# arbobendik/web-ray-tracer

Measured on AMD Instinct MI355X. Metric: Mray/s at 1080p (spp x bounces x pixels / s), higher is better.
Workload: dtype f32

## Files before the change

web-ray-tracer_amd/csrc/flx_api.hip:

```cpp
#include <hip/hip_runtime.h>

#include <chrono>
#include <sched.h>
#include <cstdio>
#include <cstdlib>
#include <algorithm>
#include <cmath>
#include <cstring>
#include <string>
#include <vector>

#include "flx_context.h"

using namespace flx;

#ifndef FLX_FRONT_FUSED_MAX_ITEMS
#define FLX_FRONT_FUSED_MAX_ITEMS (128u << 20)
#endif
#ifndef FLX_FRONT_MIN_TILES_PER_CU
#define FLX_FRONT_MIN_TILES_PER_CU 24
#endif
#ifndef FLX_ADAPTIVE_FRONT_MAX_TILES_PER_CU
#define FLX_ADAPTIVE_FRONT_MAX_TILES_PER_CU 48
#endif
// ... 196 lines not shown
  for (flx_context *c : { ctx, ctx->twin })
    if (c && c->d_frame_rings) (void)hipMemsetAsync(c->d_frame_rings, 0xff, (size_t)c->frame_rings_chains * c->prop.multiProcessorCount * WF_FRAME_RINGS * WF_FRAME_RING * sizeof(uint32_t), c->stream);
  char msg[360];
  snprintf(msg, sizeof msg, "device error in a frame kernel (bits 0x%x:%s%s%s%s%s%s%s): the frame is incomplete", bits, (bits & WF_ERR_SHADE_WATCHDOG) ? " shade-wave watchdog" : "",
           (bits & WF_ERR_WALK_WATCHDOG) ? " walk-wave watchdog" : "", (bits & WF_ERR_LIST) ? " resume list overflow" : "", (bits & WF_ERR_LEFTOVER) ? " paths left behind" : "",
           (bits & WF_ERR_RING_SLOT) ? " ring slot never filled" : "", (bits & WF_ERR_SERVER_IDLE) ? " frame server: nothing to do for seconds" : "",
           (bits & WF_ERR_SERVER_TIMEOUT) ? " frame server: no answer within 5 s" : "");
  std::string full = msg;
  if (ctx->h_sv_mail && (bits & (WF_ERR_SERVER_IDLE | WF_ERR_SERVER_TIMEOUT))) {
    char more[240];
    unsigned long long st[SV_STAT_WORDS] = {};
    if (ctx->d_sv_stats) (void)hipMemcpy(st, ctx->d_sv_stats, sizeof st, hipMemcpyDeviceToHost);
    snprintf(more, sizeof more, " [frame server: posted %u %u %u, done %u %u %u, stop after %u, next %u; launch completed %llu frames, %llu rotations, %llu tiles]", ctx->h_sv_mail->posted[0],
             ctx->h_sv_mail->posted[1], ctx->h_sv_mail->posted[2], ctx->h_sv_mail->done[0], ctx->h_sv_mail->done[1], ctx->h_sv_mail->done[2], ctx->h_sv_mail->stopAfter, ctx->sv_next_seq,
             st[SVS_FRAMES], st[SVS_ROTATIONS], st[SVS_TILES]);
    full += more;
  }
  return flx_fail(ctx, FLX_ERR_DEVICE, full.c_str());
}

static flx_status ensure_workspace(flx_context *ctx, const DeviceFrame &fr, int pipeline, bool counted, int &wf_chains) {
  const size_t P = (size_t)fr.rows * fr.width;
  const uint32_t cus = (uint32_t)ctx->prop.multiProcessorCount;
  wf_chains = 1;
  if (pipeline != 1) {
    flx_status s;
    if (path_item_count64(fr) + 1000000ull >= 4294967296ull) return fail(ctx, FLX_ERR_INVALID, "frame (or batch of frames) too large: more than 2^32 path items");
    {
      const size_t items = (size_t)path_item_count64(fr);
      struct { size_t need, have; } w[] = {
        { P, ctx->d_hits.capacity() }, { P, ctx->d_last.capacity() }, { P * (size_t)fr.samples, ctx->d_samples.capacity() },
        { pipeline == 3 ? items * 8 : 0, ctx->d_rec.capacity() }, { pipeline == 3 ? items * 3 : 0, ctx->d_rec0.capacity() },
        { pipeline == 3 ? items / (size_t)fr.samples * 3 : 0, ctx->d_pix0.capacity() } };
      size_t grow = 0, freed = 0;
      for (auto &b : w) if (b.need > b.have) { grow += b.need * sizeof(float4); freed += b.have * sizeof(float4); }
      if (pipeline == 3) {
        const size_t live = wavefront_live_capacity(fr, cus) * (size_t)(ctx->wf_groups < 1 ? 1 : (ctx->wf_groups > WF_MAX_GROUPS ? WF_MAX_GROUPS : ctx->wf_groups));
        for (auto &list : ctx->d_live) if (!list.fits(live)) { grow += live * sizeof(uint32_t); freed += list.capacity() * sizeof(uint32_t); }
      }
      size_t memFree = 0, memTotal = 0;
      if (grow && hipMemGetInfo(&memFree, &memTotal) == hipSuccess && grow > memFree + freed) {
        char msg[256];
        snprintf(msg, sizeof msg, "the path records of this frame / batch need %.1f GB of device memory, %.1f GB are free (of %.1f GB): render fewer frames per batch or a smaller frame",
                 grow / 1e9, (memFree + freed) / 1e9, memTotal / 1e9);
        return fail(ctx, FLX_ERR_DEVICE, msg);
      }
    }
    if ((s = ctx->d_hits.ensure(ctx, P))) return s;
    if ((s = ctx->d_last.ensure(ctx, P))) return s;
    if ((s = ctx->d_samples.ensure(ctx, P * (size_t)fr.samples))) return s;
  }
  if (pipeline == 3) {
    flx_status s;
    if ((s = ctx->d_rec.ensure(ctx, (size_t)path_item_count(fr) * 8))) return s;
    if ((s = ctx->d_rec0.ensure(ctx, (size_t)path_item_count(fr) * 3))) return s;
    if ((s = ctx->d_pix0.ensure(ctx, (size_t)path_item_count(fr) / (size_t)fr.samples * 3))) return s;
    wf_chains = ctx->wf_groups < 1 ? 1 : (ctx->wf_groups > WF_MAX_GROUPS ? WF_MAX_GROUPS : ctx->wf_groups);
    {
      const uint32_t tiles = path_item_count(fr) / ((uint32_t)fr.samples * 64u);
      if ((uint32_t)wf_chains > tiles || counted) wf_chains = 1;
    }
    const size_t need = wavefront_live_capacity(fr, cus) * (size_t)wf_chains;
    for (auto &list : ctx->d_live) if ((s = list.ensure(ctx, need))) return s;
  }
  return FLX_OK;
}

static flx_status angle_table(flx_context *ctx, DeviceScene &scT) {
  scT.angle_tan = nullptr;
  if (ctx->angle_table && ctx->n_entries != 0u) {
    const uint64_t key = ((uint64_t)ctx->geometry_version << 32) | ctx->transforms_version;
    if (key != ctx->angle_key || !ctx->d_angle_tan) {
      flx_status es = ctx->d_angle_tan.ensure(ctx, ctx->n_entries);
      if (es) return es;
      launch_angle_tan(scT, ctx->d_angle_tan, ctx->stream);
      FLX_HIP(ctx, hipGetLastError());
      ctx->angle_key = key;
    }
    scT.angle_tan = ctx->d_angle_tan;
  }
  return FLX_OK;
}
flx_status flx_angle_table(flx_context *ctx, DeviceScene &sc) { return angle_table(ctx, sc); }

flx_status flx_run_frame(flx_context *ctx, const DeviceScene &sc, const DeviceFrame &fr, float4 *d_out, const GBufferPtrs &gb) {
  { flx_status ss = flx_server_stop(ctx); if (ss) return ss; }
  unsigned long long *cnt = ctx->counters_enabled ? ctx->d_counters : nullptr;
  int pipeline = ctx->pipeline;
  if (pipeline == 0) {
    if (fr.use_filter || fr.is_temporal) pipeline = 1;
    else if (ctx->walk_entries <= 128u) {
      const uint64_t work = (uint64_t)fr.samples * (uint64_t)(fr.max_reflections > 0 ? fr.max_reflections : 1);
      const bool persistent = path_item_count64(fr) >= (1u << 20) && (work >= 32u || (ctx->n_lights >= 4u && work >= 4u));
      pipeline = persistent ? 2 : 1;
    } else pipeline = 3;
  }
  if (pipeline == 3 && fr.max_reflections > WF_MAX_BOUNCES) pipeline = 2;
  ctx->last_pipeline = pipeline;
  ctx->last_organisation = 0;
  ctx->last_trace = TraceKernel{ -1, -1, -1 };
  if (pipeline != 1 && (fr.use_filter || fr.is_temporal)) return fail(ctx, FLX_ERR_INVALID, "pipelines 2 and 3 do not produce the G-buffers of filter / temporal frames");
  const uint32_t cus = (uint32_t)ctx->prop.multiProcessorCount;
  int wf_chains = 1;
  { flx_status s = ensure_workspace(ctx, fr, pipeline, cnt != nullptr, wf_chains); if (s) return s; }
  FLX_HIP(ctx, hipEventRecord(ctx->ev_frame0, ctx->stream));
  if (cnt) FLX_HIP(ctx, hipMemsetAsync(cnt, 0, FLX_COUNTER_SLOTS * sizeof(unsigned long long), ctx->stream));
  if (pipeline == 1) {
    DeviceScene scT = sc;
    { flx_status es = angle_table(ctx, scT); if (es) return es; }
    FLX_HIP(ctx, hipEventRecord(ctx->ev_k0, ctx->stream));
    ctx->last_trace = launch_trace_pixels(scT, fr, d_out, gb, cnt, ctx->stream, ctx->sample_parallel);
    FLX_HIP(ctx, hipGetLastError());
    FLX_HIP(ctx, hipEventRecord(ctx->ev_k1, ctx->stream));
  } else if (pipeline == 2) {
    FLX_HIP(ctx, hipMemsetAsync(ctx->d_queue, 0, sizeof(uint32_t), ctx->stream));
    launch_primary(sc, fr, ctx->d_hits, cnt, ctx->stream);
    FLX_HIP(ctx, hipGetLastError());
    FLX_HIP(ctx, hipEventRecord(ctx->ev_k0, ctx->stream));
    DeviceScene scPaths = sc;
    if (FLX_PATHS_ANGLE_TABLE) { flx_status es = angle_table(ctx, scPaths); if (es) return es; }
    if (ctx->lock_boxes < (uint32_t)FLX_PATHS_LOCK_MIN_BOXES) scPaths.lock_entries = 0u;
    launch_paths(scPaths, fr, ctx->d_hits, ctx->d_samples, ctx->d_last, ctx->d_queue, cus * 8u, cnt, ctx->stream);
    FLX_HIP(ctx, hipGetLastError());
    FLX_HIP(ctx, hipEventRecord(ctx->ev_k1, ctx->stream));
    launch_resolve(fr, ctx->d_hits, ctx->d_samples, ctx->d_last, d_out, ctx->stream);
    FLX_HIP(ctx, hipGetLastError());
  } else {
    FLX_HIP(ctx, hipMemsetAsync(ctx->d_wfcounts, 0, WF_MAX_GROUPS * 2 * (WF_MAX_BOUNCES + 2) * sizeof(uint32_t), ctx->stream));
    { flx_status s = ctx->d_tail_pool.ensure(ctx, (size_t)WF_MAX_GROUPS * cus * 8u * WF_TAIL_POOL_F4); if (s) return s; }
    if (ctx->frame_rings_chains < wf_chains) {
      if (ctx->d_frame_rings) FLX_HIP(ctx, hipStreamSynchronize(ctx->stream));
      ctx->frame_rings_chains = 0;
      const size_t words = (size_t)wf_chains * cus * WF_FRAME_RINGS * WF_FRAME_RING;
      { flx_status s = ctx->d_frame_rings.ensure(ctx, words); if (s) return s; }
      FLX_HIP(ctx, hipMemsetAsync(ctx->d_frame_rings, 0xff, words * sizeof(uint32_t), ctx->stream));
      ctx->frame_rings_chains = wf_chains;
    }
    const int organisationNow = FLX_WF_ORGANISATION_DEFAULT ? FLX_WF_ORGANISATION_DEFAULT : ctx->wf_organisation;
    const uint32_t frameTiles = path_item_count(fr) / ((uint32_t)fr.samples * 64u);
    const int frontMode = wf_chains == 1 ? ctx->frame_front : 0;
    const bool front = (frontMode == 1 || frontMode == 2) && ctx->d_rec0 != nullptr &&
                       (frontMode == 2 || frameTiles >= (uint32_t)FLX_FRONT_MIN_TILES_PER_CU * cus) &&
                       wavefront_front_in_kernel(sc, fr, path_item_count(fr), organisationNow);
    const bool fusedFront = !front && (frontMode == 2 || frontMode == 3 || (frontMode == 1 && path_item_count(fr) <= (uint32_t)FLX_FRONT_FUSED_MAX_ITEMS));
    if (!front && !fusedFront) launch_primary(sc, fr, ctx->d_hits, cnt, ctx->stream);
    FLX_HIP(ctx, hipGetLastError());
    const uint32_t total = path_item_count(fr);
    const uint32_t perTile = (uint32_t)fr.samples * 64u;
    const uint32_t tiles = total / perTile;
    const int groups = wf_chains;
    const bool adaptive = ctx->adaptive_order && (!front || tiles < (uint32_t)FLX_ADAPTIVE_FRONT_MAX_TILES_PER_CU * cus) && groups == 1 && fr.frames <= 1u && !ctx->d_tile_order && cnt == nullptr;
    const int orderMode = 1;
    if (adaptive && !(ctx->d_tile_time.fits(tiles) && ctx->d_auto_order.fits(tiles))) {
      FLX_HIP(ctx, hipStreamSynchronize(ctx->stream));
      ctx->auto_order_tiles = 0;
      flx_status s;
      if ((s = ctx->d_tile_time.ensure(ctx, tiles)) || (s = ctx->d_auto_order.ensure(ctx, tiles))) return s;
    }
    if (adaptive && !(ctx->auto_order_tiles == tiles && ctx->auto_order_width == fr.width && ctx->auto_order_rows == fr.rows && ctx->auto_order_mode == orderMode)) {
      ctx->auto_order_tiles = 0;
      FLX_HIP(ctx, hipMemsetAsync(ctx->d_tile_time, 0, (size_t)tiles * sizeof(float), ctx->stream));
    }
    const size_t listSlice = std::min(ctx->d_live[0].capacity(), ctx->d_live[1].capacity()) / (size_t)groups;
    if (groups > 1) {
      FLX_HIP(ctx, hipEventRecord(ctx->ev_fork, ctx->stream));
      for (int g = 1; g < groups; g++) FLX_HIP(ctx, hipStreamWaitEvent(ctx->aux_stream[g - 1], ctx->ev_fork, 0));
    }
    for (int g = 0; g < groups; g++) {
      const uint32_t t0 = (uint32_t)((uint64_t)tiles * g / groups), t1 = (uint32_t)((uint64_t)tiles * (g + 1) / groups);
      WavefrontBuffers wb;
      wb.rec = ctx->d_rec; wb.rec0 = ctx->d_rec0; wb.pix0 = ctx->d_pix0;
      wb.tailPool = ctx->d_tail_pool + (size_t)g * cus * 8u * WF_TAIL_POOL_F4;
      wb.frameRings = ctx->d_frame_rings + (size_t)g * cus * WF_FRAME_RINGS * WF_FRAME_RING;
      wb.front = front ? 1u : (fusedFront ? 2u : 0u);
      wb.error = ctx->d_dev_error; wb.watchdog = ctx->inject_watchdog; wb.inject = ctx->inject_flags; wb.stampCosts = (adaptive && front) ? 1u : 0u;
      wb.tileOrder = (groups == 1 && ctx->d_tile_order && ctx->tile_order_n == tiles) ? ctx->d_tile_order : nullptr;
      if (!wb.tileOrder && adaptive && ctx->auto_order_tiles == tiles && ctx->auto_order_width == fr.width && ctx->auto_order_rows == fr.rows && ctx->auto_order_mode == orderMode)
        wb.tileOrder = ctx->d_auto_order;
      wb.tileCost = (cnt && ctx->d_tile_cost && ctx->d_tile_cost.capacity() >= tiles) ? ctx->d_tile_cost : nullptr;
      wb.tileCostPrimary = (wb.tileCost && ctx->d_tile_cost.capacity() >= 2u * tiles) ? 1u : 0u;
      wb.live[0] = ctx->d_live[0] + listSlice * g; wb.live[1] = ctx->d_live[1] + listSlice * g;
      wb.counts = ctx->d_wfcounts + (size_t)g * 2 * (WF_MAX_BOUNCES + 2); wb.walkQueue = wb.counts + (WF_MAX_BOUNCES + 2);
      wb.item_base = t0 * perTile; wb.item_count = (t1 - t0) * perTile;
      wb.hits = ctx->d_hits; wb.sampleRadiance = ctx->d_samples; wb.lastOriginal = ctx->d_last; wb.counters = cnt;
      hipStream_t st = g == 0 ? ctx->stream : ctx->aux_stream[g - 1];
      const uint32_t cusWalk = (ctx->comm && (ctx->twin || ctx->is_twin) && cus > 4u * FLX_COMM_RESERVED_CUS) ? cus - FLX_COMM_RESERVED_CUS : cus;
      WalkLdsLaunch lds;
      const int ran = launch_wavefront(sc, fr, wb, cusWalk, cnt != nullptr, organisationNow, g == 0 ? ctx->ev_k0 : nullptr, g == 0 ? ctx->ev_k1 : nullptr, st, &lds);
      FLX_HIP(ctx, hipGetLastError());
      if (ran == -2) return fail(ctx, FLX_ERR_DEVICE, "the walk kernels need 156 KB of dynamic LDS and hipFuncSetAttribute refused it on this device");
      if (ran < 0) return fail(ctx, FLX_ERR_DEVICE, "internal: the frame kernel was to trace the primary rays but does not take this frame");
      ctx->last_organisation = ran;
      ctx->last_walk_lds = lds;
      if (g > 0) {
        FLX_HIP(ctx, hipEventRecord(ctx->ev_join[g - 1], st));
        FLX_HIP(ctx, hipStreamWaitEvent(ctx->stream, ctx->ev_join[g - 1], 0));
      }
    }
    const bool measured = adaptive && ctx->last_organisation >= 2;
    launch_resolve(fr, ctx->d_hits, ctx->d_samples, ctx->d_last, d_out, ctx->stream, 0, measured ? ctx->d_tile_time : nullptr);
    FLX_HIP(ctx, hipGetLastError());
    if (measured) {
      launch_tile_order(ctx->d_tile_time, ctx->d_auto_order, tiles, orderMode, ctx->stream);
      FLX_HIP(ctx, hipGetLastError());
      ctx->auto_order_tiles = tiles; ctx->auto_order_width = fr.width; ctx->auto_order_rows = fr.rows; ctx->auto_order_mode = orderMode;
    } else if (adaptive) ctx->auto_order_tiles = 0;
  }
  FLX_HIP(ctx, hipEventRecord(ctx->ev_frame1, ctx->stream));
  ctx->timed = true;
  return FLX_OK;
}

static flx_status ensure_post_buffers(flx_context *ctx, size_t pixels, bool gbuffers, bool planes);

static flx_status run_post_frame(flx_context *ctx, const DeviceScene &sc, const DeviceFrame &fr, const flx_frame_params *p, float4 *d_out, uint32_t *planes_out = nullptr) {
  const bool temporal = fr.is_temporal == 1, filter = fr.use_filter == 1;
  if (fr.rows != fr.height && (!temporal || (filter && !planes_out)))
    return fail(ctx, FLX_ERR_INVALID, "filter frames cannot be tiled: the denoise chain reads neighbouring pixels (render the whole frame on one context)");
  const size_t pixels = (size_t)fr.rows * fr.width;
  flx_status s;
  if ((s = ensure_post_buffers(ctx, pixels, true, filter && !planes_out))) return s;
  FilterPlanes pl = {};
  if (planes_out) {
    pl.R[0] = planes_out; pl.Ip[0] = planes_out + pixels; pl.O[0] = planes_out + 2 * pixels; pl.Id[0] = planes_out + 3 * pixels; pl.OId = planes_out + 4 * pixels;
  } else if (filter) {
    for (int i = 0; i < 4; i++) { pl.R[i] = ctx->d_planes[i]; pl.Ip[i] = ctx->d_planes[4 + i]; }
    pl.O[0] = ctx->d_planes[8]; pl.O[1] = ctx->d_planes[9]; pl.Id[0] = ctx->d_planes[10]; pl.Id[1] = ctx->d_planes[11]; pl.OId = ctx->d_planes[12];
  }
  int N = 1;
  if (temporal) {
    N = p->temporal_samples <= 0 ? 4 : (p->temporal_samples > 16 ? 16 : p->temporal_samples);
    if (ctx->ring_n != N || ctx->ring_w != fr.width || ctx->ring_h != fr.height ||
        ctx->ring_tile_rows != fr.tile_rows || ctx->ring_tile_index != fr.tile_index || ctx->ring_tile_count != fr.tile_count) {
      ctx->ring_n = 0;
      for (auto &ring : ctx->d_ring) for (auto &plane : ring) if ((s = plane.release(ctx))) return s;
      for (int r = 0; r < 4; r++) for (int i = 0; i < N; i++) {
        if ((s = ctx->d_ring[r][i].ensure(ctx, pixels))) return s;
        FLX_HIP(ctx, hipMemsetAsync(ctx->d_ring[r][i], 0, pixels * sizeof(uint32_t), ctx->stream));
      }
      ctx->ring_n = N; ctx->ring_head = 0; ctx->ring_w = fr.width; ctx->ring_h = fr.height;
      ctx->ring_tile_rows = fr.tile_rows; ctx->ring_tile_index = fr.tile_index; ctx->ring_tile_count = fr.tile_count;
    }
  }
  GBufferPtrs gb = { ctx->d_gb[0], ctx->d_gb[1], ctx->d_gb[2], ctx->d_gb[3], ctx->d_gb[4], ctx->d_gb[5] };
  if (filter && !temporal && !ctx->gb_float_wanted) {
    GBufferPtrs q = { nullptr, nullptr, nullptr, nullptr, nullptr, nullptr };
    q.q_color = pl.R[0]; q.q_color_ip = pl.Ip[0]; q.q_original_color = pl.O[0]; q.q_id = pl.Id[0]; q.q_original_id = pl.OId;
    if ((s = flx_run_frame(ctx, sc, fr, nullptr, q))) return s;
    launch_filter_chain(pl, d_out, (int)fr.width, (int)fr.height, p->hdr, ctx->stream);
    FLX_HIP(ctx, hipGetLastError());
    FLX_HIP(ctx, hipEventRecord(ctx->ev_frame1, ctx->stream));
    return FLX_OK;
  }
  if ((s = flx_run_frame(ctx, sc, fr, nullptr, gb))) return s;
  if (temporal) {
    ctx->ring_head = (ctx->ring_head + N - 1) % N;
    TemporalPass t = {};
    t.color = gb.color; t.color_ip = gb.color_ip; t.location_id = gb.location_id; t.original_id = gb.original_id; t.original_color = gb.original_color; t.id = gb.id;
    for (int k = 0; k < 16; k++) {
      const int slot = (ctx->ring_head + k) % N;
      t.ring_c[k] = k < N ? ctx->d_ring[0][slot] : nullptr; t.ring_ip[k] = k < N ? ctx->d_ring[1][slot] : nullptr;
      t.ring_id[k] = k < N ? ctx->d_ring[2][slot] : nullptr; t.ring_oid[k] = k < N ? ctx->d_ring[3][slot] : nullptr;
    }
    t.n = N; t.hdr = p->hdr; t.pixels = pixels;
    if (filter) { t.dColor = pl.R[0]; t.dIp = pl.Ip[0]; t.dOColor = pl.O[0]; t.dId = pl.Id[0]; t.dOId = pl.OId; }
    else t.out = d_out;
    launch_temporal(t, ctx->stream);
  } else {
    launch_quantize(gb.color, pl.R[0], pixels, ctx->stream);
    launch_quantize(gb.color_ip, pl.Ip[0], pixels, ctx->stream);
    launch_quantize(gb.original_color, pl.O[0], pixels, ctx->stream);
// ... 524 lines not shown
    if ((s = ctx->d_sv_rings.ensure(ctx, ringWords))) return s;
    FLX_HIP(ctx, hipMemsetAsync(ctx->d_sv_rings, 0xff, ringWords * sizeof(uint32_t), ctx->stream));
    if ((s = ctx->d_sv_stats.ensure(ctx, SV_STAT_TOTAL))) return s;
    if ((s = ctx->d_sv_versions.ensure(ctx, (size_t)cus * SV_MAX_DEPTH * SV_BLOB_WORDS))) return s;
    if ((s = ctx->d_sv_slots.ensure(ctx, SV_MAX_DEPTH))) return s;
  }
  int chains = 1;
  if ((s = ensure_workspace(ctx, fr, 3, false, chains))) return s;
  const size_t P1 = (size_t)frOne.rows * frOne.width;
  if (!ctx->sv_target_slots && ctx->d_sv_out.capacity() < SV_MAX_DEPTH * P1) {
    FLX_HIP(ctx, hipStreamSynchronize(ctx->stream));
    if ((s = ctx->d_sv_out.ensure(ctx, SV_MAX_DEPTH * P1))) return s;
  }
  const size_t tilesPerSlot0 = itemsPerSlot / ((size_t)fr.samples * 64u);
  const size_t groupsMin = ctx->sv_groups && ctx->sv_groups < cus ? ctx->sv_groups : (cus > 16 ? cus - 8 : cus);
  size_t tcap = FLX_SERVER_TILE_LIST_FACTOR * (tilesPerSlot0 / groupsMin + 1);
  if (tcap < FLX_SERVER_TILE_LIST_MIN) tcap = FLX_SERVER_TILE_LIST_MIN;
  if (ctx->sv_tile_cap < tcap) {
    ctx->sv_tile_cap = 0;
    if ((s = ctx->d_sv_tiles.ensure(ctx, (size_t)cus * SV_MAX_DEPTH * tcap))) return s;
    ctx->sv_tile_cap = tcap;
  }
  if (!ctx->copy_stream) {
    FLX_HIP(ctx, hipStreamCreateWithFlags(&ctx->copy_stream, hipStreamNonBlocking));
    for (int i = 0; i < 3; i++) {
      FLX_HIP(ctx, hipEventCreate(&ctx->ev_slot_start[i]));
      FLX_HIP(ctx, hipEventCreate(&ctx->ev_slot_traced[i]));
      FLX_HIP(ctx, hipEventCreateWithFlags(&ctx->ev_slot_done[i], hipEventDisableTiming));
    }
  }
  return FLX_OK;
}

static bool server_versions_fit(const flx_context *ctx) {
  return ctx->sv_moving && ctx->have_transforms && ctx->n_transforms != 0 && server_blob_words(ctx->n_transforms, ctx->n_lights) <= SV_BLOB_WORDS &&
         ctx->h_rotation.size() == (size_t)ctx->n_transforms * 24 && ctx->h_shift.size() == (size_t)ctx->n_transforms * 8 && ctx->h_lights.size() == (size_t)ctx->n_lights * 6;
}
static bool server_continues(flx_context *ctx, const flx_frame_params *params, bool out8) {
  const uint32_t depth = ctx->frame_lanes == 3 ? 3u : 2u;
  const bool same_scene = ctx->sv_ver ? ctx->sv_structure_version == ctx->structure_version : ctx->sv_scene_version == ctx->scene_version;
  return ctx->sv_running && ctx->sv_depth == depth && chain_same_shape(ctx->sv_params, *params) && same_scene && ctx->sv_out8 == out8;
}
int flx_server_takes_moving_scene(const flx_context *ctx) { return ctx->sv_want_ver && server_versions_fit(ctx) ? 1 : 0; }
int flx_server_continues(flx_context *ctx, const flx_frame_params *params) { return server_continues(ctx, params, ctx->sv_target_slots != 0u && ctx->sv_target8) ? 1 : 0; }
flx_status flx_server_prepare(flx_context *ctx, const flx_frame_params *params) {
  FLX_HIP(ctx, hipSetDevice(ctx->device));
  DeviceScene sc; DeviceFrame fr;
  flx_status s = flx_make_frame(ctx, params, sc, fr);
  if (s) return s;
  if ((s = flx_server_stop(ctx))) return s;
  if (ctx->sv_stream) FLX_HIP(ctx, hipStreamSynchronize(ctx->sv_stream));
  if ((s = server_allocate(ctx, fr, ctx->frame_lanes == 3 ? 3u : 2u))) return s;
  FLX_HIP(ctx, hipStreamSynchronize(ctx->stream));
  return FLX_OK;
}

static flx_status server_post(flx_context *ctx, const flx_frame_params *params, const DeviceScene &sc, const DeviceFrame &frOne, uint32_t *seqOut, uint32_t *slotOut, bool out8) {
  const uint32_t cus = (uint32_t)ctx->prop.multiProcessorCount;
  const uint32_t depth = ctx->frame_lanes == 3 ? 3u : 2u;
  flx_status s;
  if (ctx->sv_running && !server_continues(ctx, params, out8))
    if ((s = server_stop(ctx))) return s;
  if (ctx->sv_running && server_idled_with_nothing_owed(ctx)) {
    ctx->sv_running = false;
    FLX_HIP(ctx, hipStreamSynchronize(ctx->sv_stream));
    __atomic_store_n(&ctx->h_dev_error[0], 0u, __ATOMIC_RELEASE);
  }
  if (!ctx->sv_running) {
    if ((s = flx_dyn_flush(ctx))) return s;
    if (ctx->sv_stream) FLX_HIP(ctx, hipStreamSynchronize(ctx->sv_stream));
    if (server_idled_with_nothing_owed(ctx)) __atomic_store_n(&ctx->h_dev_error[0], 0u, __ATOMIC_RELEASE);
    for (int i = 0; i < ctx->fifo_n; i++) {
      if (ctx->fifo[i].lane != ctx) continue;
      const int kp = ctx->fifo[i].slot;
      if (ctx->sv_pending[kp].valid && (s = server_take(ctx, kp))) return s;
    }
    DeviceFrame fr = frOne;
    fr.frames = depth; fr.rows = depth * frOne.frame_rows;
    for (uint32_t i = 0; i < depth; i++) memset(&fr.view[i], 0, sizeof(FrameView));
    const size_t itemsPerSlot = (size_t)path_item_count64(frOne);
    if ((s = server_allocate(ctx, frOne, depth))) return s;
    const size_t P1 = (size_t)frOne.rows * frOne.width;
    ctx->sv_out_pixels = P1;
    FLX_HIP(ctx, hipStreamSynchronize(ctx->stream));
    ctx->sv_counter += 16u;
    if (ctx->sv_counter < 16u) ctx->sv_counter = 16u;
    const uint32_t seq0 = ctx->sv_counter;
    memset((void *)ctx->h_sv_mail, 0, sizeof(ServerMail));
    FLX_HIP(ctx, hipMemsetAsync(ctx->d_sv_slots, 0, SV_MAX_DEPTH * sizeof(ServerSlot), ctx->sv_stream));
    FLX_HIP(ctx, hipMemsetAsync(ctx->d_sv_relay, 0, sizeof(ServerMail), ctx->sv_stream));
    FLX_HIP(ctx, hipMemsetAsync(ctx->d_sv_stats, 0, SV_STAT_TOTAL * sizeof(unsigned long long), ctx->sv_stream));
    WavefrontBuffers wb = {};
    wb.rec = ctx->d_rec; wb.rec0 = ctx->d_rec0; wb.pix0 = ctx->d_pix0;
    wb.frameRings = ctx->d_sv_rings; wb.front = 1u;
    wb.error = ctx->d_dev_error; wb.watchdog = 0u; wb.inject = 0u;
    wb.item_base = 0u; wb.item_count = (uint32_t)(depth * itemsPerSlot);
    wb.hits = ctx->d_hits; wb.sampleRadiance = ctx->d_samples; wb.lastOriginal = ctx->d_last; wb.counters = nullptr;
    ServerArgs sa = {};
    sa.slots = ctx->d_sv_slots; sa.mail = ctx->d_sv_mail; sa.relay = ctx->d_sv_relay;
    const uint32_t slot0 = ctx->sv_target_slots ? (uint32_t)(ctx->sv_target_posted % depth) : ((ctx->fifo_n && ctx->sv_depth == depth) ? ctx->sv_next_slot % depth : 0u);
    sa.depth = depth; sa.slot0 = slot0; sa.seq0 = seq0;
    sa.tilesPerSlot = (uint32_t)(itemsPerSlot / ((size_t)fr.samples * 64u));
    sa.itemsPerSlot = (uint32_t)itemsPerSlot;
    for (uint32_t i = 0; i < depth; i++) sa.out[i] = ctx->d_sv_out + (size_t)i * P1;
    if (ctx->sv_target_slots) {
      const size_t first = (size_t)params->tile_index * params->tile_rows * params->width;
      for (uint32_t i = 0; i < depth; i++) sa.out[i] = out8 ? (float4 *)((uint32_t *)ctx->sv_target[i] + first) : ctx->sv_target[i] + first;
      sa.outStripRows = params->tile_rows; sa.outStripStep = params->tile_rows * params->tile_count; sa.outSystem = 1u;
    }
    sa.out8 = out8 ? 1u : 0u;
    sa.tileLists = ctx->d_sv_tiles; sa.tileListCap = (uint32_t)ctx->sv_tile_cap;
    sa.idleExit = 200000000u;
    sa.error = ctx->d_dev_error;
    sa.stats = ctx->d_sv_stats;
    uint32_t cusWalk = cus > 4u * FLX_SERVER_RESERVED_CUS ? cus - FLX_SERVER_RESERVED_CUS : cus;
    if (ctx->sv_groups && ctx->sv_groups < cusWalk) cusWalk = ctx->sv_groups;
    const bool ver = ctx->sv_want_ver && server_versions_fit(ctx);
    DeviceScene scL = sc;
    if (ver) {
      const size_t versions = (size_t)cusWalk * depth;
      sa.blobWords = server_blob_words(ctx->n_transforms, ctx->n_lights);
      scL.rotation = (const float4 *)ctx->d_sv_versions.get();
      scL.shift = (const float4 *)(ctx->d_sv_versions + versions * ctx->n_transforms * 24u);
      scL.lights = (const float *)(ctx->d_sv_versions + versions * ctx->n_transforms * 32u);
    }
    if (launch_server(scL, fr, wb, sa, cusWalk, ctx->sv_stream, &ctx->last_walk_lds) != 0) return fail(ctx, FLX_ERR_DEVICE, "internal: the frame server does not take this scene");
    FLX_HIP(ctx, hipGetLastError());
    ctx->sv_running = true; ctx->sv_depth = depth; ctx->sv_next_seq = seq0; ctx->sv_next_slot = slot0;
    ctx->sv_params = *params; ctx->sv_scene_version = ctx->scene_version; ctx->sv_out8 = out8;
    ctx->sv_ver = ver; ctx->sv_structure_version = ctx->structure_version;
  }
  const uint32_t seq = ctx->sv_next_seq++, slot = ctx->sv_next_slot;
  ctx->sv_next_slot = (slot + 1u) % depth;
  if (ctx->sv_target_slots) ctx->sv_target_posted++;
  memcpy((void *)&ctx->h_sv_mail->view[slot], &frOne.view[0], sizeof(FrameView));
  if (ctx->sv_ver) {
    uint32_t *b = (uint32_t *)ctx->h_sv_mail->blob[slot];
    memcpy(b, ctx->h_rotation.data(), (size_t)ctx->n_transforms * 96);
    memcpy(b + (size_t)ctx->n_transforms * 24, ctx->h_shift.data(), (size_t)ctx->n_transforms * 32);
    if (ctx->n_lights) memcpy(b + (size_t)ctx->n_transforms * 32, ctx->h_lights.data(), (size_t)ctx->n_lights * 24);
  }
  __atomic_store_n(&ctx->h_sv_mail->posted[slot], seq, __ATOMIC_RELEASE);
  *seqOut = seq; *slotOut = slot;
  ctx->last_pipeline = 3; ctx->last_organisation = 5; ctx->last_chained = 3; ctx->last_trace = TraceKernel{ -1, -1, -1 };
  return FLX_OK;
}

static flx_status server_take(flx_context *ctx, int k) {
  auto &pf = ctx->sv_pending[k];
  pf.valid = false;
  ctx->slot_latency_ms[k] = -1.f;
  const auto t0 = std::chrono::steady_clock::now();
  uint32_t spins = 0;
  while (__atomic_load_n(&ctx->h_sv_mail->done[pf.slot], __ATOMIC_ACQUIRE) != pf.seq) {
    if (__atomic_load_n(&ctx->h_dev_error[0], __ATOMIC_ACQUIRE) != 0u) break;
    if ((++spins & 1023u) == 0u && std::chrono::steady_clock::now() - t0 > std::chrono::seconds(5)) {
      __atomic_fetch_or(&ctx->h_dev_error[0], WF_ERR_SERVER_TIMEOUT, __ATOMIC_RELEASE);
      break;
    }
    if (spins < 4096u) __builtin_ia32_pause(); else sched_yield();
  }
  if (server_idled_with_nothing_owed(ctx)) {
    ctx->sv_running = false;
    FLX_HIP(ctx, hipStreamSynchronize(ctx->sv_stream));
    __atomic_store_n(&ctx->h_dev_error[0], 0u, __ATOMIC_RELEASE);
  }
  if (__atomic_load_n(&ctx->h_dev_error[0], __ATOMIC_ACQUIRE) != 0u) {
    __atomic_store_n(&ctx->h_sv_mail->stopAfter, 1u, __ATOMIC_RELEASE);
    ctx->sv_running = false;
    return FLX_OK;
  }
  ctx->slot_latency_ms[k] = std::chrono::duration<float, std::milli>(std::chrono::steady_clock::now() - pf.posted).count();
  const float4 *src = ctx->sv_target_slots ? ctx->sv_target[pf.slot] : ctx->d_sv_out + (size_t)pf.slot * ctx->sv_out_pixels;
  ctx->slot_dev_ptr[k] = src;
  FLX_HIP(ctx, hipEventRecord(ctx->ev_slot_start[k], ctx->copy_stream));
  FLX_HIP(ctx, hipEventRecord(ctx->ev_slot_traced[k], ctx->copy_stream));
  if (pf.format != FLX_FRAME_DEVICE) {
    if (ctx->slot_bytes[k]) FLX_HIP(ctx, hipMemcpyAsync(ctx->h_slot[k], src, ctx->slot_bytes[k], hipMemcpyDeviceToHost, ctx->copy_stream));
    FLX_HIP(ctx, hipEventRecord(ctx->ev_slot_done[k], ctx->copy_stream));
  }
  return FLX_OK;
}

constexpr int NOT_GATHERED = -2;
struct FrameKind { bool raster = false; int aa = 0;  };
static flx_status frame_begin_on(flx_context *ctx, const flx_frame_params *params, int format, int gather, int *slot, int chained = 0 ,
                                 FrameKind kind = FrameKind()) {
  FLX_HIP(ctx, hipSetDevice(ctx->device));
  DeviceScene sc; DeviceFrame fr;
  flx_status s = flx_make_frame(ctx, params, sc, fr);
  if (s) return s;
  if (!chained) ctx->last_chained = 0;
  const bool gathered = gather != NOT_GATHERED;
  const bool receiver = !gathered || gather < 0 || gather == ctx->comm_rank;
  if (gathered) { fr.rows = receiver ? params->height : 0u; }
  const int k = (int)(ctx->frames_begun % (uint64_t)(ctx->frame_lanes == 3 ? 3 : 2));
  if (!ctx->copy_stream) {
    FLX_HIP(ctx, hipStreamCreateWithFlags(&ctx->copy_stream, hipStreamNonBlocking));
    for (int i = 0; i < 3; i++) {
      FLX_HIP(ctx, hipEventCreate(&ctx->ev_slot_start[i]));
      FLX_HIP(ctx, hipEventCreate(&ctx->ev_slot_traced[i]));
// ... 572 lines not shown
```

web-ray-tracer_amd/csrc/flx_context.h:

```cpp
#ifndef FLX_CONTEXT_H
#define FLX_CONTEXT_H

#include <hip/hip_runtime.h>

#include <chrono>
#include <cstdint>
#include <string>
#include <vector>

#include "flexlight_hip.h"
#include "flexlight_hip_debug.h"
#include "flx_kernels.h"
#include "flx_ray_temporal_args.h"
#include "flx_server.h"

struct flx_share;
typedef struct ncclComm *flx_nccl_comm;

#ifndef FLX_WF_GROUPS
#define FLX_WF_GROUPS 1
#endif
constexpr int WF_MAX_GROUPS = 4;
#ifndef FLX_SAMPLE_PARALLEL_DEFAULT
#define FLX_SAMPLE_PARALLEL_DEFAULT 1
// ... 20 lines not shown
  T *operator->() const { return p; }
  size_t capacity() const { return n; }
  bool fits(size_t count) const { return p && n >= count; }
  flx_status ensure(flx_context *ctx, size_t count, unsigned pinned_flags = 0);
  flx_status release(flx_context *ctx);
  void borrow(const Buffer &o) { (void)hip_free(); p = o.p; n = o.n; owned = false; }
 private:
  T *p = nullptr;
  size_t n = 0;
  bool owned = true;
  hipError_t hip_free() {
    T *mine = owned ? p : nullptr;
    p = nullptr; n = 0; owned = true;
    return !mine ? hipSuccess : Pinned ? hipHostFree(mine) : hipFree(mine);
  }
};
template <typename T> using DeviceBuffer = Buffer<T, false>;
template <typename T> using PinnedBuffer = Buffer<T, true>;

struct flx_context {
  int device = 0;
  hipStream_t own_stream = nullptr, stream = nullptr;
  std::string err;
  hipDeviceProp_t prop;
  DeviceBuffer<float4> d_geometry, d_attributes, d_rotation, d_shift;
  DeviceBuffer<float4> d_walk;
  uint32_t walk_entries = 0, walk_hot = 0, walk_root = 0, walk_fast_boxes = 0;
  uint32_t walk_thick_boxes = 0;
  int box_test = -1;
  DeviceBuffer<float4> d_fwd;
  uint32_t fwd_entries = 0, fwd_root = 0, lock_boxes = 0;
  int last_organisation = 0;
  flx::WalkLdsLaunch last_walk_lds;
  int frame_front = 1;
  DeviceBuffer<uint32_t> d_frame_rings;
  int frame_rings_chains = 0;
  int wf_organisation = 0;
  bool lock_ok = false;
  bool lock_use = true;
  bool gb_float_wanted = false;
  int sample_parallel = FLX_SAMPLE_PARALLEL_DEFAULT;
  int adaptive_order = 1;
  DeviceBuffer<float> d_tile_time; DeviceBuffer<uint32_t> d_auto_order;
  uint32_t auto_order_tiles = 0, auto_order_width = 0, auto_order_rows = 0; int auto_order_mode = -1;
  DeviceBuffer<uint32_t> d_tile_order; uint32_t tile_order_n = 0;
  DeviceBuffer<unsigned long long> d_tile_cost;
  DeviceBuffer<int32_t> d_ids;
  DeviceBuffer<float> d_lights;
  DeviceBuffer<uchar4> d_atlas[3];
  uint32_t atlas_w[3] = { 0, 0, 0 }, atlas_h[3] = { 0, 0, 0 };
  struct { uint32_t w = 0, h = 0, n = 0; } atlas_cells[3];
  DeviceBuffer<flx::AtlasSource> d_texture_table;
  DeviceBuffer<uint4> d_texture_src;
  DeviceBuffer<uint32_t> d_texture_cell;
  uint32_t n_entries = 0, n_ids = 0, n_transforms = 0, n_lights = 0;
  uint32_t max_transform = 0;
  bool have_scene = false, have_transforms = false, have_lights = false;
  std::vector<uint32_t> h_entry_meta;
  bool scene_has_nan = false;
  PinnedBuffer<float> h_update;
  hipEvent_t update_done = nullptr;
  bool update_pending = false;
  DeviceBuffer<float4> d_update_rows, d_update_attributes;
  DeviceBuffer<uint32_t> d_update_verdict;
  PinnedBuffer<uint32_t> h_update_verdict;
  hipStream_t update_stream = nullptr;
  hipEvent_t update_checked = nullptr, update_produced = nullptr, geometry_uploaded = nullptr;
  DeviceBuffer<uint32_t> d_refit;
  DeviceBuffer<uint32_t> d_derive;
  PinnedBuffer<uint32_t> h_derive_record;
  bool entry_meta_stale = false;
  struct {
    DeviceBuffer<float2> tbox; DeviceBuffer<uint32_t> perm[2], owner[2], open, bucket, entry, keys, verdict, refit; DeviceBuffer<uint2> x, y, totals;
    DeviceBuffer<uint4> node, cnt; DeviceBuffer<double> centre;
    size_t node_capacity = 0;
    uint32_t n_triangles = 0, n_nodes = 0; int current = 0; float transform = 0.0f; bool valid = false;
  } tree;
  PinnedBuffer<uint32_t> h_tree_record;
  DeviceBuffer<float4> d_angle_tan;
  uint64_t angle_key = ~0ull;
  uint32_t geometry_version = 0;
  uint32_t transforms_version = 0;
  int angle_table = 1;
  DeviceBuffer<float4> d_out;
  DeviceBuffer<float4> d_gb[6];
  DeviceBuffer<uint32_t> d_planes[13];
  DeviceBuffer<uint32_t> d_qbatch;
  DeviceBuffer<uint32_t> d_ring[4][16];
  int ring_n = 0, ring_head = 0;
  uint32_t ring_w = 0, ring_h = 0;
  uint32_t ring_tile_rows = 0, ring_tile_index = 0, ring_tile_count = 0;
  DeviceBuffer<float4> d_hits, d_samples, d_last;
  DeviceBuffer<uint32_t> d_queue;
  DeviceBuffer<float4> d_rec;
  DeviceBuffer<float4> d_tail_pool;
  DeviceBuffer<uint32_t> d_aa[10];
  uint32_t aa_w = 0, aa_h = 0;
  int taa_head = 0, taa_filled = 0;
  DeviceBuffer<float4> d_aa_io[2];
  DeviceBuffer<float4> d_rec0, d_pix0;
  DeviceBuffer<uint32_t> d_live[2];
  DeviceBuffer<uint32_t> d_wfcounts;
  int pipeline = 0;
  int last_pipeline = 0;
  flx::TraceKernel last_trace = { -1, -1, -1 };
  int wf_groups = FLX_WF_GROUPS;
  hipStream_t aux_stream[3] = { nullptr, nullptr, nullptr };
  hipEvent_t ev_fork = nullptr, ev_join[3] = { nullptr, nullptr, nullptr };
  PinnedBuffer<uint32_t> h_dev_error; uint32_t *d_dev_error = nullptr;
  uint32_t inject_watchdog = 0, inject_flags = 0;
  DeviceBuffer<unsigned long long> d_counters;
  bool counters_enabled = false;
  flx_counters last_counters = {};
  hipEvent_t ev_frame0 = nullptr, ev_frame1 = nullptr, ev_k0 = nullptr, ev_k1 = nullptr;
  bool timed = false;
  flx_nccl_comm comm = nullptr;
  flx_nccl_comm comm_twin = nullptr;
  int last_gather_root = -1;
  int comm_rank = 0, comm_size = 1;
  bool comm_owned = false;
  DeviceBuffer<float4> d_send, d_recv;
  DeviceBuffer<float4> d_send8;
  DeviceBuffer<float4> d_frames;
  DeviceBuffer<float4> d_gplanes;
  DeviceBuffer<float4> d_slot[3];
  DeviceBuffer<uint32_t> d_slot8[3];
  PinnedBuffer<uint8_t> h_slot[3];
  size_t slot_bytes[3] = { 0, 0, 0 };
  hipStream_t copy_stream = nullptr;
  hipEvent_t ev_slot_start[3] = {}, ev_slot_traced[3] = {}, ev_slot_done[3] = {};
  uint64_t frames_begun = 0, frames_ended = 0;
  bool slot_host[3] = { true, true, true };
  flx_context *twin = nullptr;
  bool is_twin = false;
  int frame_lanes = 2;
  uint64_t lane_next = 0;
  struct { flx_context *lane; int slot; } fifo[3] = {};
  int fifo_n = 0;
  std::vector<float> h_lights, h_rotation, h_shift;
  uint64_t dyn_version = 0, twin_dyn_version = 0;
  int frame_chain = FLX_FRAME_CHAIN_DEFAULT;
  uint64_t scene_version = 0;
  uint64_t begin_scene_version = 0;
  int last_chained = 0;
  DeviceBuffer<flx::ServerSlot> d_sv_slots;
  PinnedBuffer<flx::ServerMail> h_sv_mail; flx::ServerMail *d_sv_mail = nullptr;
  DeviceBuffer<flx::ServerMail> d_sv_relay;
  DeviceBuffer<uint32_t> d_sv_rings;
  DeviceBuffer<float4> d_sv_out;
  size_t sv_out_pixels = 0;
  DeviceBuffer<uint32_t> d_sv_tiles;
  size_t sv_tile_cap = 0;
  float slot_latency_ms[3] = { -1.f, -1.f, -1.f };
  const void *slot_dev_ptr[3] = { nullptr, nullptr, nullptr };
  DeviceBuffer<unsigned long long> d_sv_stats;
  hipStream_t sv_stream = nullptr;
  bool sv_running = false;
  uint32_t sv_depth = 0, sv_next_seq = 0, sv_next_slot = 0, sv_counter = 0;
  flx_frame_params sv_params = {};
  uint64_t sv_scene_version = 0;
  uint64_t structure_version = 0;
  uint64_t sv_structure_version = 0;
  bool sv_ver = false;
  uint32_t dyn_device_stale = 0;
  bool sv_want_ver = false;
  int sv_moving = 1;
// ... 105 lines not shown
```

web-ray-tracer_amd/csrc/flx_device.h:

```cpp
#ifndef FLX_DEVICE_H
#define FLX_DEVICE_H

#include <hip/hip_runtime.h>
#include <stdint.h>

#include "flx_math.h"

#define FLX_DEV __device__ __forceinline__

namespace flx {

constexpr float PHI = 1.61803398874989484820459f;
constexpr float SQRT3 = 1.7320508075688772f;
constexpr float INV_PI = 0.3183098861837907f;
constexpr float INV_256 = 0.00390625f;
constexpr float INV_255 = 0.00392156862745098f;
constexpr float PI_F = 3.141592653589793f;
constexpr float BIAS = FLX_BIAS;
constexpr float POW32 = FLX_POW32;
constexpr float NEAR_VIEW_DEPTH = 0.5f;

struct f3 { float x, y, z; };
struct f4 { float x, y, z, w; };
struct M3 { f3 c0, c1, c2; };

FLX_DEV f3 F3(float x, float y, float z) { f3 r; r.x = x; r.y = y; r.z = z; return r; }
FLX_DEV f3 operator+(f3 a, f3 b) { return F3(a.x + b.x, a.y + b.y, a.z + b.z); }
FLX_DEV f3 operator-(f3 a, f3 b) { return F3(a.x - b.x, a.y - b.y, a.z - b.z); }
FLX_DEV f3 operator*(f3 a, f3 b) { return F3(a.x * b.x, a.y * b.y, a.z * b.z); }
FLX_DEV f3 operator/(f3 a, f3 b) { return F3(a.x / b.x, a.y / b.y, a.z / b.z); }
FLX_DEV f3 operator*(f3 a, float s) { return F3(a.x * s, a.y * s, a.z * s); }
FLX_DEV f3 operator/(f3 a, float s) { return F3(a.x / s, a.y / s, a.z / s); }
FLX_DEV f3 operator-(f3 a) { return F3(-a.x, -a.y, -a.z); }
FLX_DEV float dot(f3 a, f3 b) { return (a.x * b.x + a.y * b.y) + a.z * b.z; }
FLX_DEV f3 cross(f3 a, f3 b) { return F3(a.y * b.z - b.y * a.z, a.z * b.x - b.z * a.x, a.x * b.y - b.x * a.y); }
FLX_DEV float length(f3 a) { return flx_sqrt(dot(a, a)); }
FLX_DEV f3 normalize(f3 a) { return a / length(a); }
FLX_DEV float distance(f3 a, f3 b) { return length(a - b); }
FLX_DEV f3 mix(f3 a, f3 b, float t) { return F3(flx_mix(a.x, b.x, t), flx_mix(a.y, b.y, t), flx_mix(a.z, b.z, t)); }
FLX_DEV f3 mul(const M3 &m, f3 v) {
  return F3((m.c0.x * v.x + m.c1.x * v.y) + m.c2.x * v.z,
            (m.c0.y * v.x + m.c1.y * v.y) + m.c2.y * v.z,
            (m.c0.z * v.x + m.c1.z * v.y) + m.c2.z * v.z);
}
FLX_DEV f3 reflect(f3 I, f3 N) { return I - N * (2.0f * dot(N, I)); }
FLX_DEV f3 refract(f3 I, f3 N, float eta) {
  float d = dot(N, I);
  float k = 1.0f - eta * eta * (1.0f - d * d);
  if (k < 0.0f) return F3(0.0f, 0.0f, 0.0f);
  return I * eta - N * (eta * d + flx_sqrt(k));
}

struct Ray { f3 origin, dir; };
struct Material { f3 albedo, rme, tpo; };
struct Hit { f3 suv; int transformId; int triangleId; };

struct DeviceScene {
  const float4 *geometry;
  const float4 *attributes;
  const float4 *rotation;
  const float4 *shift;
  const float *lights;
  const uchar4 *atlas[3];
  uint32_t atlas_w[3], atlas_h[3];
  uint32_t n_entries;
  uint32_t n_lights;
  uint32_t n_transforms;
  uint32_t walk_thick_boxes;
  const float4 *walk;
  uint32_t walk_entries;
  uint32_t walk_hot;
  uint32_t walk_root;
  uint32_t walk_fast_boxes;
  const float4 *lock;
  uint32_t lock_entries;
  uint32_t lock_root;
  const float4 *fwd;
  uint32_t fwd_entries, fwd_root;
  const float4 *angle_tan;
};
#ifndef FLX_LOCKSTEP
#define FLX_LOCKSTEP 1
#endif
#define FLX_LOCK_MAX 128u
constexpr uint32_t WALK_END = 0x30000000u;
constexpr uint32_t LINK_INDEX = 0x0fffffffu, LINK_XFORM = 0x40000000u;
constexpr int LINK_KIND_SHIFT = 28;
FLX_DEV uint32_t linkIndex(uint32_t link) { return link & LINK_INDEX; }
FLX_DEV uint32_t linkKind(uint32_t link) { return (link >> LINK_KIND_SHIFT) & 3u; }
// ... 172 lines not shown
  if (!(s < l) || !(s * viewDepthPerS >= NEAR_VIEW_DEPTH)) return false;
  suv = F3(s, u, v);
  return s != 0.0f;
}

FLX_DEV bool rayCuboid(float l, const Ray &ray, f3 minCorner, f3 maxCorner) {
  f3 v0 = (minCorner - ray.origin) / ray.dir;
  f3 v1 = (maxCorner - ray.origin) / ray.dir;
  float tmin = flx_max(flx_max(flx_min(v0.x, v1.x), flx_min(v0.y, v1.y)), flx_min(v0.z, v1.z));
  float tmax = flx_min(flx_min(flx_max(v0.x, v1.x), flx_max(v0.y, v1.y)), flx_max(v0.z, v1.z));
  return tmax >= flx_max(tmin, BIAS) && tmin < l;
}

FLX_DEV float trowbridgeReitz(float alpha, float NdotH) {
  float numerator = alpha * alpha;
  float denom = NdotH * NdotH * (numerator - 1.0f) + 1.0f;
  return numerator / flx_max(PI_F * denom * denom, BIAS);
}
FLX_DEV float schlickBeckmann(float alpha, float NdotX) {
  float k = alpha * 0.5f;
  float denominator = NdotX * (1.0f - k) + k;
  denominator = flx_max(denominator, BIAS);
  return NdotX / denominator;
}
FLX_DEV float smith(float alpha, float NdotV, float NdotL) { return schlickBeckmann(alpha, NdotV) * schlickBeckmann(alpha, NdotL); }
FLX_DEV f3 fresnel(f3 F0, float theta) {
  float p = flx_pow5(1.0f - theta);
  return F3(F0.x + (1.0f - F0.x) * p, F0.y + (1.0f - F0.y) * p, F0.z + (1.0f - F0.z) * p);
}

FLX_DEV f3 forwardTrace(const Material &material, f3 lightDir, float strength, f3 N, f3 V) {
  float lenP1 = 1.0f + length(lightDir);
  float brightness = strength / (lenP1 * lenP1);
  f3 L = normalize(lightDir);
  f3 H = normalize(V + L);
  float VdotH = flx_max(dot(V, H), 0.0f);
  float NdotL = flx_max(dot(N, L), 0.0f);
  float NdotH = flx_max(dot(N, H), 0.0f);
  float NdotV = flx_max(dot(N, V), 0.0f);
  float alpha = material.rme.x * material.rme.x;
  float BRDF = flx_mix(1.0f, NdotV, material.rme.y);
  f3 F0 = material.albedo * BRDF;
  f3 Ks = fresnel(F0, VdotH);
  float oneMinusMetal = 1.0f - material.rme.y;
  f3 Kd = F3((1.0f - Ks.x) * oneMinusMetal, (1.0f - Ks.y) * oneMinusMetal, (1.0f - Ks.z) * oneMinusMetal);
  f3 lambert = material.albedo * INV_PI;
  float tr = trowbridgeReitz(alpha, NdotH);
  float sm = smith(alpha, NdotV, NdotL);
  f3 cookTorranceNumerator = (Ks * tr) * sm;
  float cookTorranceDenominator = 4.0f * NdotV * NdotL;
  cookTorranceDenominator = flx_max(cookTorranceDenominator, BIAS);
  f3 cookTorrance = cookTorranceNumerator / cookTorranceDenominator;
  f3 radiance = Kd * lambert + cookTorrance;
  return (radiance * NdotL) * brightness;
}

struct PixelState {
  float firstRayLength, glassFilter, originalRMEx, originalTPOx;
  f3 originalColor;
  f4 renderId, renderOriginalId;
  float ndc_x, ndc_y;
  float seed;
  uint32_t lightBase = 0;
};

struct PathState {
  Ray ray;
  f3 lastHitPoint;
  f3 finalColor, importancyFactor;
  Hit hit;
  bool dontFilter;
};

struct ShadeOut {
  f3 litColor;
  f3 baseLuminance;
  Ray shadowRay;
  float shadowLen;
  bool needShadow;
  bool shadowedNoWalk;
  bool markId;
};

FLX_DEV void reservoirPick(const DeviceScene &sc, const DeviceFrame &fr, PixelState &ps, const Material &material, const Ray &ray,
                           f4 randomVec, f3 N, f3 smoothNormal, float geometryOffset, bool dontFilter, int i, ShadeOut &so) {
  f3 localColor = F3(0.0f, 0.0f, 0.0f);
  float reservoirLength = 0.0f;
  float totalWeight = 0.0f;
  int reservoirNum = 0;
  float reservoirWeight = 0.0f;
  f3 reservoirLightDir = F3(0.0f, 0.0f, 0.0f);
  f4 n0 = noise(ps.seed, randomVec.z, randomVec.w, BIAS);
  float lastRandomX = n0.x, lastRandomY = n0.y;
  const int size = (int)sc.n_lights;
  for (int j = 0; j < size; j++) {
    const float *lt = sc.lights + 6 * j + ps.lightBase;
    float strength = lt[3], variation = lt[4];
    if (strength <= 0.0f) continue;
    reservoirLength += 1.0f;
    f3 light = F3(lt[0], lt[1], lt[2]) + F3(randomVec.x, randomVec.y, randomVec.z) * variation;
    f3 dir = light - ray.origin;
    f3 colorForLight = forwardTrace(material, dir, strength, N, -ray.dir);
    localColor = localColor + colorForLight;
    float weight = length(colorForLight);
    totalWeight += weight;
    if (flx_abs(lastRandomY) * totalWeight <= weight) {
      reservoirNum = j;
      reservoirWeight = weight;
      reservoirLightDir = dir;
    }
    if (j + 1 < size) {
      f4 n1 = noise(ps.seed, lastRandomX, lastRandomY, BIAS);
      lastRandomX = n1.z; lastRandomY = n1.w;
    }
  }
  f3 unitLightDir = normalize(reservoirLightDir);
  bool showColor = reservoirLength == 0.0f || reservoirWeight == 0.0f;
  bool showShadow = dot(smoothNormal, unitLightDir) <= BIAS;
  so.baseLuminance = F3(material.rme.z, material.rme.z, material.rme.z);
  so.litColor = localColor + so.baseLuminance;
  so.markId = dontFilter || i == 0;
  if (so.markId) ps.renderId.w = (float)((reservoirNum % 128) << 1) * INV_255;
  so.needShadow = !showColor && !showShadow;
  so.shadowedNoWalk = !showColor && showShadow;
  so.shadowRay.origin = ray.origin + smoothNormal * geometryOffset;
  so.shadowRay.dir = unitLightDir;
  so.shadowLen = length(reservoirLightDir);
}

struct SurfaceCtx {
  f3 origin;
  f3 dir;
  f3 smoothNormal;
  float signDir, geometryOffset, BRDF, roughnessBRDF;
  f3 F0;
  Material material;
};

#ifndef FLX_ANGLE_TABLE
#define FLX_ANGLE_TABLE 0
#endif
FLX_DEV f3 triangleAngleTan(f3 t0v, f3 t1v, f3 t2v, f3 n0, f3 n1, f3 n2) {
  f3 geometryNormal = normalize(cross(t0v - t1v, t0v - t2v));
  f3 angles = F3(flx_acos(flx_abs(dot(geometryNormal, n0))), flx_acos(flx_abs(dot(geometryNormal, n1))),
                 flx_acos(flx_abs(dot(geometryNormal, n2))));
  return F3(flx_clamp(flx_tan(angles.x), 0.0f, 1.0f), flx_clamp(flx_tan(angles.y), 0.0f, 1.0f),
            flx_clamp(flx_tan(angles.z), 0.0f, 1.0f));
}
FLX_DEV f3 triangleAngleTanOf(const DeviceScene &sc, int tri) {
  const float4 g0 = sc.geometry[3 * tri], g1 = sc.geometry[3 * tri + 1], g2 = sc.geometry[3 * tri + 2];
  const M3 rTI = rotation_at(sc, (int)g2.y << 1);
  const float4 *at = sc.attributes + 7 * (size_t)tri;
  const float4 a0 = at[0], a1 = at[1], a2 = at[2];
  return triangleAngleTan(mul(rTI, F3(g0.x, g0.y, g0.z)), mul(rTI, F3(g0.w, g1.x, g1.y)), mul(rTI, F3(g1.z, g1.w, g2.x)),
                          mul(rTI, F3(a0.x, a0.y, a0.z)), mul(rTI, F3(a0.w, a1.x, a1.y)), mul(rTI, F3(a1.z, a1.w, a2.x)));
}

template <bool COUNT>
FLX_DEV void shadeSurface(const DeviceScene &sc, const DeviceFrame &fr, const Hit &hit, const Ray &ray, f3 lastHitPoint, SurfaceCtx &sf,
                          WorkCounters &cnt) {
  if (COUNT) cnt.shades++;
  M3 rTI = rotation_at(sc, hit.transformId);
  f3 sTI = shift_at(sc, hit.transformId);
  sf.origin = ray.dir * hit.suv.x + ray.origin;
  f3 uvw = F3(1.0f - hit.suv.y - hit.suv.z, hit.suv.y, hit.suv.z);
  float4 g0 = sc.geometry[3 * hit.triangleId], g1 = sc.geometry[3 * hit.triangleId + 1], g2 = sc.geometry[3 * hit.triangleId + 2];
  f3 t0v = mul(rTI, F3(g0.x, g0.y, g0.z));
  f3 t1v = mul(rTI, F3(g0.w, g1.x, g1.y));
  f3 t2v = mul(rTI, F3(g1.z, g1.w, g2.x));
  f3 offsetRayTarget = sf.origin - sTI;
  f3 diffs = F3(distance(offsetRayTarget, t0v), distance(offsetRayTarget, t1v), distance(offsetRayTarget, t2v));
  const float4 *at = sc.attributes + 7 * (size_t)hit.triangleId;
  float4 a0 = at[0], a1 = at[1], a2 = at[2], a3 = at[3], a4 = at[4], a5 = at[5], a6 = at[6];
  f3 n0 = mul(rTI, F3(a0.x, a0.y, a0.z));
  f3 n1 = mul(rTI, F3(a0.w, a1.x, a1.y));
  f3 n2 = mul(rTI, F3(a1.z, a1.w, a2.x));
  f3 smoothNormal = normalize(F3((n0.x * uvw.x + n1.x * uvw.y) + n2.x * uvw.z,
                                 (n0.y * uvw.x + n1.y * uvw.y) + n2.y * uvw.z,
                                 (n0.z * uvw.x + n1.z * uvw.y) + n2.z * uvw.z));
  f3 angleTan;
  if (FLX_ANGLE_TABLE && sc.angle_tan) { const float4 t = sc.angle_tan[hit.triangleId]; angleTan = F3(t.x, t.y, t.z); }
  else angleTan = triangleAngleTan(t0v, t1v, t2v, n0, n1, n2);
  sf.geometryOffset = dot(diffs * angleTan, uvw);
  float bu = (a2.y * uvw.x + a2.w * uvw.y) + a3.y * uvw.z;
  float bv = (a2.z * uvw.x + a3.x * uvw.y) + a3.z * uvw.z;
  sf.material.albedo = fetchTexVal<COUNT>(sc, fr, 0, bu, bv, a3.w, F3(a4.z, a4.w, a5.x), cnt);
  sf.material.rme = fetchTexVal<COUNT>(sc, fr, 1, bu, bv, a4.x, F3(a5.y, a5.z, a5.w), cnt);
  sf.material.tpo = fetchTexVal<COUNT>(sc, fr, 2, bu, bv, a4.y, F3(a6.x, a6.y, a6.z), cnt);

  sf.dir = normalize(sf.origin - lastHitPoint);
  sf.signDir = flx_sign(dot(sf.dir, smoothNormal));
  sf.smoothNormal = smoothNormal * (-sf.signDir);
  sf.BRDF = flx_mix(1.0f, flx_abs(dot(sf.smoothNormal, sf.dir)), sf.material.rme.y);
  sf.roughnessBRDF = sf.material.rme.x * sf.BRDF;
  sf.F0 = sf.material.albedo * sf.BRDF;
}

FLX_DEV void shadeSample(const DeviceScene &sc, const DeviceFrame &fr, const SurfaceCtx &sf, PixelState &ps, PathState &p, f3 camera, float cosSampleN,
                         int i, ShadeOut &so) {
  const float fi = (float)i;
  const Material &material = sf.material;
  const f3 smoothNormal = sf.smoothNormal;
  p.ray.origin = sf.origin;
  p.ray.dir = sf.dir;
  f4 randomVec = noise(ps.seed, ps.ndc_x, ps.ndc_y, fi + cosSampleN);
  f3 randomSpheareVec = normalize(smoothNormal + normalize(F3(randomVec.x, randomVec.y, randomVec.z)));
  f3 roughNormal = normalize(mix(smoothNormal, randomSpheareVec, sf.roughnessBRDF));
  f3 H = normalize(roughNormal - p.ray.dir);
  float VdotH = flx_max(dot(-p.ray.dir, H), 0.0f);
  f3 f = fresnel(sf.F0, VdotH);
  float fresnelReflect = flx_max(f.x, flx_max(f.y, f.z));
  bool isSolid = material.tpo.x * fresnelReflect <= flx_abs(randomVec.w);

  if (p.dontFilter) {
    ps.originalTPOx = material.tpo.x;
    ps.originalColor = ps.originalColor * material.albedo;
    ps.originalRMEx += material.rme.x;
    if (fr.use_filter) {
      float scale = flx_exp2_neg_int(i);
      f3 cn = combineNormalRME(smoothNormal, material.rme);
      f4 upd; upd.x = scale * cn.x; upd.y = scale * cn.y; upd.z = scale * cn.z; upd.w = scale * 0.0f;
      ps.renderId.x += upd.x; ps.renderId.y += upd.y; ps.renderId.z += upd.z; ps.renderId.w += upd.w;
      if (i == 0) {
        ps.renderOriginalId.x += upd.x; ps.renderOriginalId.y += upd.y; ps.renderOriginalId.z += upd.z; ps.renderOriginalId.w += upd.w;
      }
    }
    p.dontFilter = (material.rme.x < 0.01f && isSolid) || !isSolid;
    if (isSolid && material.tpo.x > 0.01f) {
      ps.glassFilter += 1.0f;
      p.dontFilter = false;
    }
  } else {
    p.importancyFactor = p.importancyFactor * material.albedo;
  }

  if (i == 1) ps.firstRayLength = flx_min(length(p.ray.origin - p.lastHitPoint) / length(p.lastHitPoint - camera), ps.firstRayLength);
  reservoirPick(sc, fr, ps, material, p.ray, randomVec, roughNormal * (-sf.signDir), smoothNormal * (-sf.signDir), sf.geometryOffset, p.dontFilter, i, so);
  if (isSolid) {
    p.ray.dir = normalize(mix(reflect(p.ray.dir, smoothNormal), randomSpheareVec, sf.roughnessBRDF));
  } else {
    float eta = flx_mix(1.0f / material.tpo.z, material.tpo.z, flx_max(sf.signDir, 0.0f));
    p.ray.dir = normalize(mix(refract(p.ray.dir, smoothNormal, eta), randomSpheareVec, sf.roughnessBRDF));
  }
}

template <bool COUNT>
FLX_DEV void bounceShade(const DeviceScene &sc, const DeviceFrame &fr, PixelState &ps, PathState &p, f3 camera, float cosSampleN, int i,
                         ShadeOut &so, WorkCounters &cnt) {
  SurfaceCtx sf;
  shadeSurface<COUNT>(sc, fr, p.hit, p.ray, p.lastHitPoint, sf, cnt);
  shadeSample(sc, fr, sf, ps, p, camera, cosSampleN, i, so);
}

#ifndef FLX_BOX_FALLBACK_COUNT
#define FLX_BOX_FALLBACK_COUNT 0
#endif
struct WalkState {
  Ray src;
  Ray tR;
  float minLen;
  int i;
  int cachedTI;
  int mode;
  int shadowed;
  f3 suv;
  int tri, hitTI;
  f3 inv;
  bool fastDiv;
#if FLX_BOX_FALLBACK_COUNT
  mutable uint32_t boxTests, boxExact;
#endif
};

FLX_DEV void walkStart(WalkState &w, int mode, const Ray &ray, float len) {
  w.mode = mode; w.src = ray; w.tR = ray; w.cachedTI = 0; w.minLen = len; w.i = 0;
}
FLX_DEV void walkClearResults(WalkState &w) {
  w.inv = F3(0.0f, 0.0f, 0.0f); w.fastDiv = false;
  w.shadowed = false; w.suv = F3(0.0f, 0.0f, 0.0f); w.tri = -1; w.hitTI = 0;
}

template <bool COUNT>
FLX_DEV bool walkStep(const DeviceScene &sc, WalkState &w, WorkCounters &cnt) {
  bool endWalk = false;
  const int i = w.i;
  float4 e0 = sc.geometry[3 * i], e1 = sc.geometry[3 * i + 1], e2 = sc.geometry[3 * i + 2];
  if (COUNT) { if (w.mode == 0) cnt.shadow_visits++; else cnt.closest_visits++; }
  int tI = (int)e2.y << 1;
  if (tI != w.cachedTI) {
    int iI = tI + 1;
    M3 rotationII = rotation_at(sc, iI);
    w.cachedTI = tI;
    w.tR.origin = mul(rotationII, w.src.origin + shift_at(sc, iI));
    f3 d = mul(rotationII, w.src.dir);
    w.tR.dir = (w.mode == 0) ? normalize(d) : d;
  }
  int next = i + 1;
  if (e2.z == 0.0f) {
    endWalk = true;
  } else if (e2.z == 1.0f) {
    if (!rayCuboid(w.minLen, w.tR, F3(e0.x, e0.y, e0.z), F3(e0.w, e1.x, e1.y))) next += (int)e1.z;
  } else {
    f3 a = F3(e0.x, e0.y, e0.z), b = F3(e0.w, e1.x, e1.y), c = F3(e1.z, e1.w, e2.x);
    if (w.mode == 0) {
      if (moellerTrumboreCull(a, b, c, w.tR, w.minLen)) { w.shadowed = true; endWalk = true; }
    } else {
      f3 suv;
      if (moellerTrumbore(a, b, c, w.tR, w.minLen, suv)) {
        w.suv = suv; w.hitTI = tI; w.tri = i;
        w.minLen = suv.x;
      }
    }
  }
  w.i = next;
  return endWalk || next >= (int)sc.n_entries;
}

struct WalkEntry { float4 e0, e1, e2; };


FLX_DEV float divByRecip(float a, float d, float y) {
  float q = a * y;
  float r = __builtin_fmaf(-q, d, a);
  q = __builtin_fmaf(r, y, q);
  r = __builtin_fmaf(-q, d, a);
  return __builtin_fmaf(r, y, q);
}
FLX_DEV void reciprocalOfDir(const DeviceScene &sc, f3 d, f3 o, f3 &inv, bool &fast) {
  inv = F3(recipFast(d.x), recipFast(d.y), recipFast(d.z));
  const float LO = 8.673617379884035e-19f, HI = 1.152921504606847e18f, OHI = 5.764607523034235e17f;
  const float ax = flx_abs(d.x), ay = flx_abs(d.y), az = flx_abs(d.z);
  fast = sc.walk_fast_boxes != 0u && ax >= LO && ax <= HI && ay >= LO && ay <= HI && az >= LO && az <= HI &&
         flx_abs(o.x) <= OHI && flx_abs(o.y) <= OHI && flx_abs(o.z) <= OHI;
}
// ... 584 lines not shown
```

web-ray-tracer_amd/csrc/flx_frame_common.h:

```cpp
#pragma once
#include "flx_kernels.h"
#include "flx_kernel_util.h"
#include "flx_wavefront_common.h"

namespace flx {

#ifndef FLX_WF_WALK_THREADS
#define FLX_WF_WALK_THREADS 1024
#endif
#ifndef FLX_WF_WAVES_PER_EU
#define FLX_WF_WAVES_PER_EU 4
#endif
#ifndef FLX_WF_LDS_TOTAL
#define FLX_WF_LDS_TOTAL (156 * 1024)
#endif
#ifndef FLX_WF_INNER
#define FLX_WF_INNER 8
#endif
#ifndef FLX_WF_UNROLL
#define FLX_WF_UNROLL 8
#endif
#ifndef FLX_WF_BATCH
#define FLX_WF_BATCH 24
#endif
#ifndef FLX_WF_DRAWS_PER_WAVE
#define FLX_WF_DRAWS_PER_WAVE 16
#endif
#ifndef FLX_FRAME_SHADERS_FRONT
#define FLX_FRAME_SHADERS_FRONT 4
#endif
#ifndef FLX_WF_MAX_TRANSFORMS
#define FLX_WF_MAX_TRANSFORMS 4
#endif
#ifndef FLX_FRAME_PROLOGUE_WAVES
#define FLX_FRAME_PROLOGUE_WAVES 2
#endif
#ifndef FLX_FRAME_READY_UNITS
#define FLX_FRAME_READY_UNITS 32
#endif

typedef const __attribute__((address_space(4))) FrameArgs *FrameArgsP;
FLX_DEV const FrameArgs &frame_args(FrameArgsP p) { asm volatile("" : "+s"(p)); return *(const FrameArgs *)p; }
FLX_DEV FrameArgsP kernel_frame_args() { return (FrameArgsP)__builtin_amdgcn_kernarg_segment_ptr(); }
#define FLX_ARGS_OF(ab) const FrameArgs &A_ = frame_args(ab); const DeviceScene &sc = A_.sc; const DeviceFrame &fr = A_.fr; const WavefrontBuffers &wb = A_.wb; (void)sc; (void)fr; (void)wb

template <bool VER>
FLX_DEV uint32_t scene_version_of(const DeviceFrame &fr, uint32_t frameIdx) { return VER ? blockIdx.x * fr.frames + frameIdx : 0u; }

template <bool COUNT, bool LV = false, bool VER = false>
FLX_DEV bool shade0_tile(FrameArgsP ab, uint32_t tile, uint32_t lane, float4 h, WorkCounters &cnt, const FrameView *lv = nullptr) {
  uint32_t S, frameIdx, lightBase = 0;
  int tri;
  bool alive, compact;
  f3 camera;
  SurfaceCtx sf;
  float ndcX = 0.0f, ndcY = 0.0f;
  Hit hit;
  {
  FLX_ARGS_OF(ab);
  S = (uint32_t)fr.samples;
  uint32_t px, k;
  tile8_pixel(fr, tile, lane, px, k);
  const bool inFrame = px < fr.width && k < fr.rows;
  frameIdx = inFrame ? frame_index(fr, k) : 0u;
  camera = view_camera(view_at<LV>(fr, lv, frameIdx));
  tri = inFrame ? __float_as_int(h.w) : -1;
  alive = tri != -1 && fr.max_reflections > 0 && length(F3(1.0f, 1.0f, 1.0f) * F3(1.0f, 1.0f, 1.0f)) >= fr.min_importancy * SQRT3;
  hit.suv = F3(h.x, h.y, h.z); hit.triangleId = tri; hit.transformId = 0;
  compact = wb.rec0 != nullptr;
  if (alive) {
    hit.transformId = (int)sc.geometry[3 * tri + 2].y << 1;
    if (VER) { const uint32_t ver = scene_version_of<VER>(fr, frameIdx); hit.transformId += (int)(ver * 2u * sc.n_transforms); lightBase = ver * 6u * sc.n_lights; }
    const uint32_t py_gl = fr.height - 1u - image_row(fr, k);
    float viewDepthPerS;
    Ray pr;
    pr.origin = camera;
    pr.dir = primary_dir_v(fr, view_at<LV>(fr, lv, frameIdx), px, py_gl, ndcX, ndcY, viewDepthPerS);
    const WorkCounters before = cnt;
    shadeSurface<COUNT>(sc, fr, hit, pr, camera, sf, cnt);
    if (COUNT) {
      cnt.shades = before.shades + (cnt.shades - before.shades) * S;
      cnt.atlas_texels = before.atlas_texels + (cnt.atlas_texels - before.atlas_texels) * S;
    }
  }
  }
  for (uint32_t s = 0; s < S; s++) {
    FLX_ARGS_OF(ab);
    const uint32_t pathId = ((tile * S + s) << 6) | lane;
    float4 *rec = wb.rec + (size_t)pathId * 8;
    if (!alive) {
      if (tri != -1) finalize_path<LV>(fr, wb, pathId, F3(0.0f, 0.0f, 0.0f), F3(1.0f, 1.0f, 1.0f), F3(1.0f, 1.0f, 1.0f), lv);
      if (compact) wb.rec0[(size_t)pathId * 3] = make_float4(0.f, 0.f, 0.f, __int_as_float(RF_DEAD));
      else rec[0] = make_float4(0.f, 0.f, 0.f, __int_as_float(RF_DEAD));
      continue;
    }
    PathState p;
    PixelState ps;
    ps.firstRayLength = 1.0f; ps.glassFilter = 0.0f; ps.originalRMEx = 0.0f; ps.originalTPOx = 0.0f;
    ps.renderId.x = ps.renderId.y = ps.renderId.z = ps.renderId.w = 0.0f;
    ps.renderOriginalId = ps.renderId;
    ps.ndc_x = ndcX; ps.ndc_y = ndcY;
    ps.seed = view_at<LV>(fr, lv, frameIdx).random_seed;
    ps.lightBase = lightBase;
    ps.originalColor = F3(1.0f, 1.0f, 1.0f);
    p.hit = hit;
    p.lastHitPoint = camera;
    p.dontFilter = true;
    p.importancyFactor = F3(1.0f, 1.0f, 1.0f);
    const float cosSampleN = flx_cos((float)s);
    ShadeOut so;
    shadeSample(sc, fr, sf, ps, p, camera, cosSampleN, 0, so);
    const int flags = (p.dontFilter ? RF_DONT_FILTER : 0) | (so.needShadow ? RF_NEED_SHADOW : 0) | (so.shadowedNoWalk ? RF_SHADOWED_NO_WALK : 0) |
                      (nextBounceRuns(fr, 0, p.importancyFactor, ps.originalColor) ? 0 : RF_NO_CLOSEST);
    if (compact) {
      if (s == 0u) {
        float4 *pp = wb.pix0 + (((size_t)tile << 6) | lane) * 3;
        pp[0] = make_float4(p.ray.origin.x, p.ray.origin.y, p.ray.origin.z, 0.0f);
        pp[1] = make_float4(so.shadowRay.origin.x, so.shadowRay.origin.y, so.shadowRay.origin.z, 0.0f);
        pp[2] = make_float4(ps.originalColor.x, ps.originalColor.y, ps.originalColor.z, so.baseLuminance.x);
      }
      float4 *r0 = wb.rec0 + (size_t)pathId * 3;
      r0[0] = make_float4(p.ray.dir.x, p.ray.dir.y, p.ray.dir.z, __int_as_float(flags));
      r0[1] = make_float4(so.shadowRay.dir.x, so.shadowRay.dir.y, so.shadowRay.dir.z, so.shadowLen);
      r0[2] = make_float4(so.litColor.x, so.litColor.y, so.litColor.z, 0.0f);
      continue;
    }
    rec[0] = make_float4(p.ray.origin.x, p.ray.origin.y, p.ray.origin.z, __int_as_float(flags));
    rec[1] = make_float4(p.ray.dir.x, p.ray.dir.y, p.ray.dir.z, so.shadowLen);
    rec[2] = make_float4(so.shadowRay.origin.x, so.shadowRay.origin.y, so.shadowRay.origin.z, so.baseLuminance.x);
    rec[3] = make_float4(so.shadowRay.dir.x, so.shadowRay.dir.y, so.shadowRay.dir.z, __int_as_float(0));
    rec[4] = make_float4(so.litColor.x, so.litColor.y, so.litColor.z, 0.0f);
    rec[5] = make_float4(0.0f, 0.0f, 0.0f, 0.0f);
    rec[6] = make_float4(p.importancyFactor.x, p.importancyFactor.y, p.importancyFactor.z, 0.0f);
    rec[7] = make_float4(ps.originalColor.x, ps.originalColor.y, ps.originalColor.z, 0.0f);
  }
  return alive;
}

template <bool COUNT, bool LV = false, bool VER = false>
FLX_DEV float4 primary_tile(FrameArgsP ab, uint32_t tile, uint32_t lane, WorkCounters &cnt, const FrameView *lv = nullptr) {
  FLX_ARGS_OF(ab);
  float4 *__restrict__ hits = const_cast<float4 *>(wb.hits);
  uint32_t px, k;
  tile8_pixel(fr, tile, lane, px, k);
  const bool inImage = px < fr.width && k < fr.rows;
  float nx, ny, viewDepthPerS = 0.0f;
  Ray pr; pr.origin = F3(0.0f, 0.0f, 0.0f); pr.dir = F3(0.0f, 0.0f, 1.0f);
  int xfBase = 0;
  if (inImage) {
    const uint32_t py_gl = fr.height - 1u - image_row(fr, k);
    const uint32_t frameIdx = frame_index(fr, k);
    if (VER) xfBase = (int)(scene_version_of<VER>(fr, frameIdx) * 2u * sc.n_transforms);
    const FrameView &v = view_at<LV>(fr, lv, frameIdx);
    pr.dir = primary_dir_v(fr, v, px, py_gl, nx, ny, viewDepthPerS);
    pr.origin = view_camera(v);
  }
  const uint32_t visitsBefore = cnt.primary_visits;
  const Hit hp = primaryWalkF(sc, inImage, pr, viewDepthPerS, cnt.primary_visits, xfBase);
  if (COUNT && wb.tileCost && wb.tileCostPrimary) {
    const uint32_t nTiles = ((fr.width + 7u) >> 3) * ((fr.rows + 7u) >> 3);
    atomicAdd(wb.tileCost + nTiles + tile, (unsigned long long)(cnt.primary_visits - visitsBefore));
  }
  float4 h = make_float4(hp.suv.x, hp.suv.y, hp.suv.z, __int_as_float(inImage ? hp.triangleId : -1));
  if (inImage) {
    if (COUNT && hp.triangleId != -1) cnt.primary_hits++;
    hits[(size_t)k * fr.width + px] = h;
  }
  return h;
}

template <bool COUNT, bool LV = false, bool VER = false>
FLX_DEV void shade_path(FrameArgsP ab, uint32_t pathId, WorkCounters &cnt, const FrameView *lv = nullptr) {
  FLX_ARGS_OF(ab);
  float4 *rec = wb.rec + (size_t)pathId * 8;
  uint32_t px, k, s;
  item_pixel(fr, pathId, px, k, s);
  const uint32_t frameIdx = frame_index(fr, k);
  const f3 camera = view_camera(view_at<LV>(fr, lv, frameIdx));
  PathState p;
  PixelState ps;
  ps.firstRayLength = 1.0f; ps.glassFilter = 0.0f; ps.originalRMEx = 0.0f; ps.originalTPOx = 0.0f;
  ps.renderId.x = ps.renderId.y = ps.renderId.z = ps.renderId.w = 0.0f;
  ps.renderOriginalId = ps.renderId;
  const float4 q0 = rec[0], q1 = rec[1], q2 = rec[2], q3 = rec[3], q6 = rec[6], q7 = rec[7];
  const int pb = __float_as_int(q3.w) + 1;
  p.ray.origin = F3(q0.x, q0.y, q0.z);
  p.lastHitPoint = p.ray.origin;
  p.ray.dir = F3(q1.x, q1.y, q1.z);
  p.hit.suv = F3(q2.x, q2.y, q2.z);
  p.hit.triangleId = __float_as_int(q2.w);
  p.hit.transformId = (int)sc.geometry[3 * p.hit.triangleId + 2].y << 1;
  if (VER) { const uint32_t ver = scene_version_of<VER>(fr, frameIdx); p.hit.transformId += (int)(ver * 2u * sc.n_transforms); ps.lightBase = ver * 6u * sc.n_lights; }
  p.dontFilter = (__float_as_int(q0.w) & RF_DONT_FILTER) != 0;
  p.importancyFactor = F3(q6.x, q6.y, q6.z);
  ps.originalColor = F3(q7.x, q7.y, q7.z);
  const uint32_t py_gl = fr.height - 1u - image_row(fr, k);
  float viewDepthPerS;
  (void)primary_dir_v(fr, view_at<LV>(fr, lv, frameIdx), px, py_gl, ps.ndc_x, ps.ndc_y, viewDepthPerS);
  ps.seed = view_at<LV>(fr, lv, frameIdx).random_seed;
  const float cosSampleN = flx_cos((float)s);
  ShadeOut so;
  bounceShade<COUNT>(sc, fr, ps, p, camera, cosSampleN, pb, so, cnt);
  const int flags = (p.dontFilter ? RF_DONT_FILTER : 0) | (so.needShadow ? RF_NEED_SHADOW : 0) | (so.shadowedNoWalk ? RF_SHADOWED_NO_WALK : 0) |
                    (nextBounceRuns(fr, pb, p.importancyFactor, ps.originalColor) ? 0 : RF_NO_CLOSEST);
  rec[0] = make_float4(p.ray.origin.x, p.ray.origin.y, p.ray.origin.z, __int_as_float(flags));
  rec[1] = make_float4(p.ray.dir.x, p.ray.dir.y, p.ray.dir.z, so.shadowLen);
  rec[2] = make_float4(so.shadowRay.origin.x, so.shadowRay.origin.y, so.shadowRay.origin.z, so.baseLuminance.x);
  rec[3] = make_float4(so.shadowRay.dir.x, so.shadowRay.dir.y, so.shadowRay.dir.z, __int_as_float(pb));
  rec[4] = make_float4(so.litColor.x, so.litColor.y, so.litColor.z, 0.0f);
  rec[6] = make_float4(p.importancyFactor.x, p.importancyFactor.y, p.importancyFactor.z, 0.0f);
  rec[7] = make_float4(ps.originalColor.x, ps.originalColor.y, ps.originalColor.z, 0.0f);
}

struct WalkLane {
  int st;
  uint32_t pathId; int flags; int pathBounce; float base;
  Ray nextRay, shadowRay; float shadowLen;
  WalkState w; WalkEntry cur;
  uint32_t v0;
};
FLX_DEV void walkLaneInit(WalkLane &L) {
  L.v0 = 0u;
  L.st = P_EMPTY; L.pathId = 0; L.flags = 0; L.pathBounce = 0; L.base = 0.0f;
  L.nextRay.origin = F3(0.f, 0.f, 0.f); L.nextRay.dir = L.nextRay.origin;
  L.shadowRay = L.nextRay; L.shadowLen = 0.0f;
  walkClearResults(L.w);
  L.w.src = L.nextRay; L.w.tR = L.nextRay; L.w.minLen = 0.0f; L.w.i = 0; L.w.cachedTI = 0;
  L.w.mode = 2;
  L.cur.e0 = L.cur.e1 = L.cur.e2 = make_float4(0.f, 0.f, 0.f, 0.f);
}
FLX_DEV const float4 *pix_part(const DeviceFrame &fr, const WavefrontBuffers &wb, uint32_t id) {
  uint32_t tile0, s0;
  item_tile(fr, id, tile0, s0);
  return wb.pix0 + (((size_t)tile0 << 6) | (id & 63u)) * 3;
}
#ifndef FLX_WF_FOLD_EARLY
#define FLX_WF_FOLD_EARLY 1
#endif
#if FLX_WF_FOLD_EARLY
struct WalkFold { float4 q4, q5, q6, q7; bool compact; };
#define FLX_WALK_LANE_FOLD_FETCH(fr_, wb_, compactRecs_, L_, F_)                                                                 \
  do {                                                                                                                           \
    const float4 *a4_ = (wb_).rec + (size_t)(L_).pathId * 8 + 4, *a7_ = a4_ + 3;                                                 \
    (F_).compact = (compactRecs_) && (L_).pathBounce == 0;                                                                       \
    if ((F_).compact) { a4_ = (wb_).rec0 + (size_t)(L_).pathId * 3 + 2; a7_ = pix_part(fr_, wb_, (L_).pathId) + 2; }             \
     \
    (F_).q4 = *a4_; (F_).q7 = *a7_;                                                                                              \
    if (!(F_).compact) { (F_).q5 = a4_[1]; (F_).q6 = a4_[2]; }       \
  } while (0)
#define FLX_WALK_LANE_FOLD_WITH(LV_, fr_, wb_, compactRecs_, L_, F_, lv_, toShade_, ended_, costed_, stamp_)                     \
  do {                                                                                                                           \
    float4 *rec_ = (wb_).rec + (size_t)(L_).pathId * 8;                                                                          \
    const bool compact_ = (F_).compact;                                                                                          \
    const float4 q4_ = (F_).q4, q7_ = (F_).q7;                                                                                   \
    float4 q5_ = make_float4(0.0f, 0.0f, 0.0f, 0.0f), q6_ = make_float4(1.0f, 1.0f, 1.0f, 0.0f);                                 \
    if (!compact_) { q5_ = (F_).q5; q6_ = (F_).q6; }                                                                             \
    const bool shadowed_ = ((L_).flags & RF_SHADOWED_NO_WALK) || (((L_).flags & RF_NEED_SHADOW) && (L_).w.shadowed);            \
    const f3 localColor_ = shadowed_ ? F3((L_).base, (L_).base, (L_).base) : F3(q4_.x, q4_.y, q4_.z);                            \
    const f3 importancy_ = F3(q6_.x, q6_.y, q6_.z), originalColor_ = F3(q7_.x, q7_.y, q7_.z);                                    \
    const f3 finalColor_ = F3(q5_.x, q5_.y, q5_.z) + localColor_ * importancy_;                                                  \
     \
    const float cost_ = (costed_) ? q5_.w + (float)(((stamp_) - ((uint32_t)(L_).flags >> 8)) & 0xffffffu) : 1.0f;      \
    bool cont_ = (L_).w.tri != -1;                                                                                               \
    if (cont_) cont_ = ((L_).pathBounce + 1) < (fr_).max_reflections && length(importancy_ * originalColor_) >= (fr_).min_importancy * SQRT3;      \
    if (cont_) {                                                                                                                 \
      if (compact_) {                                         \
                                                                            \
        rec_[0] = make_float4((L_).nextRay.origin.x, (L_).nextRay.origin.y, (L_).nextRay.origin.z, __int_as_float((L_).flags & 0xff));             \
        rec_[1] = make_float4((L_).nextRay.dir.x, (L_).nextRay.dir.y, (L_).nextRay.dir.z, (L_).shadowLen);                                         \
        rec_[3] = make_float4((L_).shadowRay.dir.x, (L_).shadowRay.dir.y, (L_).shadowRay.dir.z, __int_as_float(0));                                \
        rec_[6] = make_float4(1.0f, 1.0f, 1.0f, 0.0f);                                                                           \
        rec_[7] = make_float4(q7_.x, q7_.y, q7_.z, 0.0f);                                                                        \
      }                                                                                                                          \
      rec_[5] = make_float4(finalColor_.x, finalColor_.y, finalColor_.z, (costed_) ? cost_ : 0.0f);                                                 \
      rec_[2] = make_float4((L_).w.suv.x, (L_).w.suv.y, (L_).w.suv.z, __int_as_float((L_).w.tri));                               \
      toShade_ = true;                                                                                                           \
    } else {                                                                                                                     \
      finalize_path<LV_>(fr_, wb_, (L_).pathId, finalColor_, importancy_, originalColor_, lv_, cost_);                           \
      ended_ = true;                                                                                                             \
    }                                                                                                                            \
    (L_).st = P_EMPTY;                                                                                                           \
  } while (0)
#define FLX_WALK_LANE_FOLD(LV_, fr_, wb_, compactRecs_, L_, lv_, toShade_, ended_, costed_, stamp_)                              \
  do {                                                                                                                           \
    WalkFold fold_;                                                                                                              \
// ... 194 lines not shown
```

web-ray-tracer_amd/csrc/flx_kernels.h:

```cpp
#ifndef FLX_KERNELS_H
#define FLX_KERNELS_H

#include "flx_device.h"

#ifndef FLX_PATHS_ANGLE_TABLE
#define FLX_PATHS_ANGLE_TABLE 1
#endif
#define FLX_FAST_BOX_BOUND 5.764607523034235e17f
namespace flx {

struct GBufferPtrs {
  float4 *color, *color_ip, *original_color, *id, *original_id, *location_id;
  uint32_t *q_color = nullptr, *q_color_ip = nullptr, *q_original_color = nullptr, *q_id = nullptr, *q_original_id = nullptr;
};

struct TraceKernel { int samples, lockstep, counted; };
TraceKernel launch_trace_pixels(const DeviceScene &sc, const DeviceFrame &fr, float4 *out, const GBufferPtrs &gb,
                                unsigned long long *counters, hipStream_t stream, int sample_parallel = 0);
uint32_t path_item_count(const DeviceFrame &fr);
uint64_t path_item_count64(const DeviceFrame &fr);
void launch_primary(const DeviceScene &sc, const DeviceFrame &fr, float4 *hits, unsigned long long *counters, hipStream_t stream);
void launch_paths(const DeviceScene &sc, const DeviceFrame &fr, const float4 *hits, float4 *sampleRadiance, float4 *lastOriginal,
                  uint32_t *queue, uint32_t blocks, unsigned long long *counters, hipStream_t stream);
void launch_resolve(const DeviceFrame &fr, const float4 *hits, const float4 *sampleRadiance, const float4 *lastOriginal, float4 *out,
                    hipStream_t stream, size_t sampleStride = 0, float *tileTime = nullptr);
void launch_tile_order(float *tileTime, uint32_t *order, uint32_t n, int mode, hipStream_t stream);
constexpr int WF_MAX_BOUNCES = 250;
struct WavefrontBuffers {
  float4 *rec;
  uint32_t *live[2];
  uint32_t *counts;
  uint32_t *walkQueue;
  uint32_t item_base, item_count;
  const float4 *hits;
  float4 *sampleRadiance, *lastOriginal;
  unsigned long long *counters;
  float4 *tailPool;
  float4 *rec0, *pix0;
  uint32_t *frameRings;
  uint32_t front;
  uint32_t *error;
  uint32_t watchdog;
  uint32_t inject;
  uint32_t stampCosts;
  uint32_t tileCostPrimary;
  const uint32_t *tileOrder;
  unsigned long long *tileCost;
};
struct FrameArgs { DeviceScene sc; DeviceFrame fr; WavefrontBuffers wb; };
constexpr uint32_t WF_FRAME_RING = 16384;
constexpr uint32_t WF_ERR_SHADE_WATCHDOG = 1u, WF_ERR_WALK_WATCHDOG = 2u, WF_ERR_LIST = 4u, WF_ERR_LEFTOVER = 8u, WF_ERR_RING_SLOT = 16u, WF_ERR_SERVER_IDLE = 32u, WF_ERR_SERVER_TIMEOUT = 64u;
constexpr uint32_t WF_INJECT_NO_SHADING = 1u;
constexpr uint32_t WF_FRAME_RINGS = 3;
constexpr size_t WF_TAIL_POOL_F4 = 1024 * 8;
size_t wavefront_live_capacity(const DeviceFrame &fr, uint32_t compute_units);
bool wavefront_front_in_kernel(const DeviceScene &sc, const DeviceFrame &fr, uint32_t item_count, int organisation);
struct WalkLdsLaunch { uint32_t ldsCount = 0, pre = 0, kind = 0, nTransforms = 0; int boxTest = -1; };
int launch_wavefront(const DeviceScene &sc, const DeviceFrame &fr, const WavefrontBuffers &wb, uint32_t compute_units, bool count,
                     int organisation, hipEvent_t walk0_begin, hipEvent_t walk0_end, hipStream_t stream, WalkLdsLaunch *ran = nullptr);
struct FilterPlanes { uint32_t *R[4], *Ip[4], *O[2], *Id[2], *OId; };
void launch_fxaa(const uint32_t *plane, float4 *out, int W, int H, hipStream_t stream);
void launch_taa(const uint32_t *const planes[9], float4 *out, int W, int H, hipStream_t stream);
void launch_fxaa(const uint32_t *plane, uint32_t *out8, int W, int H, hipStream_t stream);
void launch_taa(const uint32_t *const planes[9], uint32_t *out8, int W, int H, hipStream_t stream);
void launch_quantize(const float4 *src, uint32_t *dst, size_t n, hipStream_t stream);
void launch_angle_tan(const DeviceScene &sc, float4 *out, hipStream_t stream);
void launch_filter_chain(const FilterPlanes &pl, float4 *out, int W, int H, int hdr, hipStream_t stream);
struct TemporalPass {
  const float4 *color, *color_ip, *location_id, *original_id, *original_color, *id;
  uint32_t *ring_c[16], *ring_ip[16], *ring_id[16], *ring_oid[16];
  int n, hdr;
  size_t pixels;
  float4 *out;
  uint32_t *dColor, *dIp, *dOColor, *dId, *dOId;
};
void launch_temporal(const TemporalPass &pass, hipStream_t stream);
void launch_raster(const DeviceScene &sc, const DeviceFrame &fr, int hdr, float4 *out, unsigned long long *counters, hipStream_t stream);
void launch_raster(const DeviceScene &sc, const DeviceFrame &fr, int hdr, uint32_t *out8, hipStream_t stream);
void launch_scene_rows(const float4 *rows, float4 *geometry, uint32_t first, uint32_t n_rows, hipStream_t stream);
void launch_rows_check_stage(const float4 *rows, const float4 *attributes, const float4 *geometry, uint32_t first, uint32_t n_rows, float4 *stage_rows,
                             float4 *stage_attributes, uint32_t *verdict, hipStream_t stream);
size_t refit_workspace_words(uint32_t n_entries);
void launch_refit(float4 *geometry, uint32_t n_entries, uint32_t *work, hipStream_t stream);
void launch_rederive(const float4 *geometry, uint32_t n_entries, float4 *copy, uint32_t entries, hipStream_t stream);
constexpr uint32_t DERIVE_RECORD_WORDS = 8;
size_t derive_workspace_words(uint32_t n_entries);
hipError_t launch_derive_check(const float4 *geometry, uint32_t n_entries, uint32_t *work, hipStream_t stream);
void launch_derive_copies(const float4 *geometry, uint32_t n_entries, uint32_t live, uint32_t *work, float4 *walk, float4 *fwd, hipStream_t stream);
void launch_entry_meta(const float4 *geometry, uint32_t n_entries, uint32_t *out, hipStream_t stream);
size_t scan_totals_items(uint32_t m);
void launch_exclusive_scan(uint2 *x, uint32_t m, uint2 *totals, hipStream_t stream);
struct TreeArrays {
  float2 *tbox; uint32_t *perm, *permNext, *owner, *ownerNext, *open, *bucket, *entry; uint2 *x, *y, *totals;
  uint4 *node, *cnt; uint32_t *keys; double *centre;
};
void launch_tree_check(const float4 *rows, uint32_t n, uint32_t *verdict, const TreeArrays &t, hipStream_t stream);
void launch_tree_level(const TreeArrays &t, uint32_t n, uint32_t base, uint32_t m, uint32_t depth, double maxDepth, hipStream_t stream);
void launch_tree_children(const TreeArrays &t, uint32_t n, uint32_t base, uint32_t m, hipStream_t stream);
void launch_tree_index(const TreeArrays &t, uint32_t n, uint32_t nodes, hipStream_t stream);
void launch_tree_emit(const float4 *rows, const float4 *attributes, const TreeArrays &t, uint32_t n, uint32_t nodes, float transform, float4 *geometry,
                      float4 *attributesOut, int32_t *ids, hipStream_t stream);
enum { SPLICE_REC_VERDICT = 0, SPLICE_REC_END, SPLICE_REC_IDS_BELOW, SPLICE_REC_IDS_ABOVE, SPLICE_RECORD_WORDS };
struct SpliceShape { uint32_t first, n_old, n_new, parent, end_new, n_padded; };
void launch_splice_check(const float4 *geometry, uint32_t n_entries, const int32_t *ids, uint32_t n_ids, uint32_t first, uint32_t n_old, uint32_t parent, uint32_t *record,
                         hipStream_t stream);
void launch_splice_rows(const float4 *geometry, const float4 *attributes, const float4 *blockGeometry, const float4 *blockAttributes, const SpliceShape &shape,
                        float4 *geometryOut, float4 *attributesOut, hipStream_t stream);
void launch_splice_ids(const int32_t *ids, uint32_t n_ids, const int32_t *blockIds, uint32_t n_block, uint32_t below, uint32_t above, uint32_t first, int32_t delta,
                       int32_t *out, hipStream_t stream);
enum { ATLAS_RGBA8 = 0, ATLAS_RGBA32F = 1 };
struct AtlasSource { const void *pixels; uint32_t sw, sh, format, pad; };
constexpr uint32_t ATLAS_TABLE_IMAGES = 2048;
void launch_atlas_cells(uint32_t *dst, uint32_t pitch, uint32_t w, uint32_t h, uint32_t tw, uint32_t first_cell, uint32_t n, const AtlasSource *table,
                        const AtlasSource *one, hipStream_t stream);
constexpr uint32_t QUERY_CHUNK = 128;
struct QueryLaunch { uint32_t ldsCount = 0, pre = 0, groups = 0, n = 0, what = 0; };
bool launch_ray_query(const DeviceScene &sc, const float4 *rays, float4 *hits, uint32_t n, uint32_t what, uint32_t *ctl, uint32_t compute_units, uint32_t groups,
                      hipStream_t stream, QueryLaunch *ran);
void launch_debug_math(int fn, const float *a, const float *b, float *out, uint32_t n, hipStream_t stream);
void launch_debug_intersect(int fn, const float *in, float *out, uint32_t n, hipStream_t stream);
bool launch_debug_walk(int variant, const DeviceScene &sc, const float *in, float *out, uint32_t n, hipStream_t stream);
bool launch_debug_walk_staged(const DeviceScene &sc, uint32_t ldsCount, const float *in, float *out, uint32_t n, hipStream_t stream);

}
#endif
```

web-ray-tracer_amd/csrc/flx_kernels.hip:

```cpp
#define FLX_SINCOS_TABLE 1
#define FLX_ANGLE_TABLE 1
#include "flx_kernels.h"
#include "flx_kernel_util.h"

#include <mutex>

#ifndef FLX_PRIMARY_FWD
#define FLX_PRIMARY_FWD 1
#endif

namespace flx {

#ifndef FLX_TRACE_BLOCK
#define FLX_TRACE_BLOCK 256
#endif
__device__ __forceinline__ void tile_pixel(const DeviceFrame &fr, uint32_t &px, uint32_t &k) {
  const uint32_t tiles_x = (fr.width + 15u) >> 4;
  const uint32_t tile = FLX_TRACE_BLOCK == 256 ? blockIdx.x : blockIdx.x >> 2;
  const uint32_t tx = tile % tiles_x, ty = tile / tiles_x;
  const uint32_t wave = FLX_TRACE_BLOCK == 256 ? threadIdx.x >> 6 : blockIdx.x & 3u, lane = threadIdx.x & 63u;
  px = (tx << 4) + ((wave & 1u) << 3) + (lane & 7u);
  k = (ty << 4) + ((wave >> 1) << 3) + (lane >> 3);
}

// ... 475 lines not shown
  if ((fr.width & 7u) == 0u) {
    cost += __shfl_xor(cost, 1); cost += __shfl_xor(cost, 2); cost += __shfl_xor(cost, 4);
    if ((threadIdx.x & 7u) == 0u && o < P && cost != 0.0f) atomicAdd(tileTime + tile, cost);
  } else if (o < P && cost != 0.0f) atomicAdd(tileTime + tile, cost);
}

#define FLX_DEV_K __device__ __forceinline__
constexpr uint32_t TO_THREADS = 512, TO_BINS = 2048, TO_CLASSES = 16, TO_BPT = TO_BINS / TO_THREADS;
FLX_DEV_K uint32_t to_bin(float c) { return c > 0.0f ? (__float_as_uint(c) >> 20) & (TO_BINS - 1u) : 0u; }
FLX_DEV_K uint32_t to_block_scan(uint32_t v, uint32_t *waveTotals , uint32_t t) {
  const uint32_t lane = t & 63u, wave = t >> 6;
  for (uint32_t d = 1; d < 64u; d <<= 1) { const uint32_t u = __shfl_up(v, d); if (lane >= d) v += u; }
  if (lane == 63u) waveTotals[wave] = v;
  __syncthreads();
  uint32_t before = 0;
  for (uint32_t w = 0; w < wave; w++) before += waveTotals[w];
  __syncthreads();
  return v + before;
}
__global__ __launch_bounds__(TO_THREADS) void k_tile_order(float *__restrict__ tileTime, uint32_t *__restrict__ order, uint32_t n, int mode) {
  __shared__ uint32_t hist[TO_BINS];
  __shared__ uint8_t binClass[TO_BINS];
  __shared__ uint16_t counts[TO_CLASSES * TO_THREADS];
  __shared__ uint32_t offs[TO_CLASSES * TO_THREADS];
  __shared__ uint32_t waveTotals[TO_THREADS / 64u];
  const uint32_t t = threadIdx.x;
  for (uint32_t b = t; b < TO_BINS; b += TO_THREADS) hist[b] = 0u;
  for (uint32_t j = t; j < TO_CLASSES * TO_THREADS; j += TO_THREADS) counts[j] = 0;
  __syncthreads();
  for (uint32_t i = t; i < n; i += TO_THREADS) atomicAdd(&hist[to_bin(tileTime[i])], 1u);
  __syncthreads();
  {
    uint32_t h[TO_BPT], sum = 0;
    for (uint32_t k = 0; k < TO_BPT; k++) { h[k] = hist[TO_BPT * t + k]; sum += h[k]; }
    uint32_t below = to_block_scan(sum, waveTotals, t) - sum;
    for (uint32_t k = 0; k < TO_BPT; k++) {
      uint32_t c;
      if (mode == 0) c = (below + h[k]) * 10u <= n ? 1u : 0u;
      else { c = (uint32_t)(((uint64_t)below * TO_CLASSES) / (n ? n : 1u)); c = TO_CLASSES - 1u - (c < TO_CLASSES ? c : TO_CLASSES - 1u); }
      binClass[TO_BPT * t + k] = (uint8_t)c;
      below += h[k];
    }
  }
  __syncthreads();
  const uint32_t chunk = (n + TO_THREADS - 1u) / TO_THREADS, lo = t * chunk < n ? t * chunk : n, hi = lo + chunk < n ? lo + chunk : n;
  for (uint32_t i = lo; i < hi; i++) counts[(uint32_t)binClass[to_bin(tileTime[i])] * TO_THREADS + t]++;
  __syncthreads();
  {
    uint32_t sum = 0;
    for (uint32_t k = 0; k < TO_CLASSES; k++) sum += counts[t * TO_CLASSES + k];
    const uint32_t incl = to_block_scan(sum, waveTotals, t);
    uint32_t at = incl - sum;
    for (uint32_t k = 0; k < TO_CLASSES; k++) { offs[t * TO_CLASSES + k] = at; at += counts[t * TO_CLASSES + k]; }
  }
  __syncthreads();
  for (uint32_t i = lo; i < hi; i++) {
    const uint32_t c = binClass[to_bin(tileTime[i])];
    order[offs[c * TO_THREADS + t]++] = i;
    tileTime[i] = 0.0f;
  }
}
void launch_tile_order(float *tileTime, uint32_t *order, uint32_t n, int mode, hipStream_t stream) {
  if (n) hipLaunchKernelGGL(k_tile_order, dim3(1), dim3(TO_THREADS), 0, stream, tileTime, order, n, mode);
}

__global__ __launch_bounds__(256) void k_angle_tan(DeviceScene sc, float4 *__restrict__ out) {
  const uint32_t i = blockIdx.x * 256u + threadIdx.x;
  if (i >= sc.n_entries) return;
  float4 r = make_float4(0.0f, 0.0f, 0.0f, 0.0f);
  const float kind = sc.geometry[3 * (size_t)i + 2].z;
  if (kind != 0.0f && kind != 1.0f) {
    const f3 t = triangleAngleTanOf(sc, (int)i);
    r = make_float4(t.x, t.y, t.z, 0.0f);
  }
  out[i] = r;
}
void launch_angle_tan(const DeviceScene &sc, float4 *out, hipStream_t stream) {
  if (sc.n_entries == 0u) return;
  DeviceScene s = sc;
  s.angle_tan = nullptr;
  hipLaunchKernelGGL(k_angle_tan, dim3((sc.n_entries + 255u) / 256u), dim3(256), 0, stream, s, out);
}

uint64_t path_item_count64(const DeviceFrame &fr) {
  return (uint64_t)((fr.width + 7u) >> 3) * ((fr.rows + 7u) >> 3) * (uint64_t)fr.samples * 64u;
}
uint32_t path_item_count(const DeviceFrame &fr) { return (uint32_t)path_item_count64(fr); }

void launch_primary(const DeviceScene &sc, const DeviceFrame &fr, float4 *hits, unsigned long long *counters, hipStream_t stream) {
  const uint32_t tiles = ((fr.width + 7u) >> 3) * ((fr.rows + 7u) >> 3);
  const uint32_t blocks = (tiles + 3u) / 4u;
  if (counters) hipLaunchKernelGGL(k_primary<true>, dim3(blocks), dim3(256), 0, stream, sc, fr, hits, counters);
  else hipLaunchKernelGGL(k_primary<false>, dim3(blocks), dim3(256), 0, stream, sc, fr, hits, counters);
}

void launch_paths(const DeviceScene &sc, const DeviceFrame &fr, const float4 *hits, float4 *sampleRadiance, float4 *lastOriginal,
                  uint32_t *queue, uint32_t blocks, unsigned long long *counters, hipStream_t stream) {
  const uint32_t total = path_item_count(fr);
  const bool lock = FLX_LOCKSTEP && sc.lock_entries != 0u;
  PathsArgs pa;
  pa.sc = sc; pa.fr = fr;
  if (FLX_PATHS_KERNARG && !FLX_PATHS_ANGLE_TABLE) pa.sc.angle_tan = nullptr;
  if (lock) {
    if (counters) hipLaunchKernelGGL((k_paths<true, true>), dim3(blocks), dim3(256), 0, stream, pa, hits, sampleRadiance, lastOriginal, queue, total, counters);
    else hipLaunchKernelGGL((k_paths<false, true>), dim3(blocks), dim3(256), 0, stream, pa, hits, sampleRadiance, lastOriginal, queue, total, counters);
  } else {
    if (counters) hipLaunchKernelGGL((k_paths<true, false>), dim3(blocks), dim3(256), 0, stream, pa, hits, sampleRadiance, lastOriginal, queue, total, counters);
    else hipLaunchKernelGGL((k_paths<false, false>), dim3(blocks), dim3(256), 0, stream, pa, hits, sampleRadiance, lastOriginal, queue, total, counters);
  }
}

void launch_resolve(const DeviceFrame &fr, const float4 *hits, const float4 *sampleRadiance, const float4 *lastOriginal, float4 *out,
                    hipStream_t stream, size_t sampleStride, float *tileTime) {
  const size_t P = (size_t)fr.rows * fr.width;
  hipLaunchKernelGGL(k_resolve, dim3((uint32_t)((P + 255) / 256)), dim3(256), 0, stream, fr, hits, sampleRadiance, lastOriginal, out, sampleStride ? sampleStride : P, tileTime);
}

__global__ void k_debug_math(int fn, const float *__restrict__ a, const float *__restrict__ b, float *__restrict__ out, uint32_t n) {
  uint32_t i = blockIdx.x * blockDim.x + threadIdx.x;
  if (i >= n) return;
  float x = a[i], y = b ? b[i] : 0.0f, r;
  switch (fn) {
    case 0: r = flx_sin(x); break;
    case 1: r = flx_cos(x); break;
    case 2: r = flx_tan(x); break;
    case 3: r = flx_acos(x); break;
    case 4: r = flx_atan2(x, y); break;
    case 5: r = flx_exp(x); break;
    case 6: r = flx_pow(x, y); break;
    case 7: r = flx_tanh(x); break;
    case 8: r = flx_floor(x); break;
    case 9: r = flx_sqrt(x); break;
    case 10: r = x / y; break;
    default: r = flx_nanf(); break;
  }
  out[i] = r;
}

__global__ void k_debug_intersect(int fn, const float *__restrict__ in, float *__restrict__ out, uint32_t n) {
  const uint32_t i = blockIdx.x * blockDim.x + threadIdx.x;
  if (i >= n) return;
  DeviceScene sc = {};
  sc.walk_fast_boxes = (fn == 6 || fn == 8) ? 0u : 1u;
  if (fn == 2 || fn >= 5) {
    const float *r = in + (size_t)i * 13u;
    WalkState w;
    w.tR.origin = F3(r[1], r[2], r[3]); w.tR.dir = F3(r[4], r[5], r[6]);
    reciprocalOfDir(sc, w.tR.dir, w.tR.origin, w.inv, w.fastDiv);
    const f3 lo = F3(r[7], r[8], r[9]), hi = F3(r[10], r[11], r[12]);
    out[i] = (fn >= 7 ? rayCuboidFast<true>(r[0], w, lo, hi) : fn != 5 ? rayCuboidFast(r[0], w, lo, hi) : rayCuboid(r[0], w.tR, lo, hi)) ? 1.0f : 0.0f;
    return;
  }
  const float *r = in + (size_t)i * 16u;
  const f3 a = F3(r[0], r[1], r[2]), b = F3(r[3], r[4], r[5]), c = F3(r[6], r[7], r[8]);
  Ray ray; ray.origin = F3(r[9], r[10], r[11]); ray.dir = F3(r[12], r[13], r[14]);
  const float l = r[15];
  f3 suv = F3(0.0f, 0.0f, 0.0f);
  bool hit;
  switch (fn) {
    case 0: hit = moellerTrumboreAny(a, b - a, c - a, ray, l, false, suv); break;
    case 1: hit = moellerTrumboreAny(a, b - a, c - a, ray, l, true, suv); break;
    case 3: hit = moellerTrumbore(a, b, c, ray, l, suv); break;
    default: hit = moellerTrumboreCull(a, b, c, ray, l); break;
  }
  if (fn == 0 || fn == 3) {
    float *o = out + (size_t)i * 3u;
// ... 147 lines not shown
```

web-ray-tracer_amd/csrc/flx_server.hip:

```cpp
#include <cstddef>
#include <cstdio>
#include <mutex>
#include "flx_server.h"
#include "flx_frame_common.h"

namespace flx {

#ifndef FLX_SERVER_RELAY_GROUPS
#define FLX_SERVER_RELAY_GROUPS 16
#endif
#ifndef FLX_SERVER_SHADERS
#define FLX_SERVER_SHADERS FLX_FRAME_SHADERS_FRONT
#endif
#ifndef FLX_SERVER_SHADERS_DEPTH2_MAX_TILES
#define FLX_SERVER_SHADERS_DEPTH2_MAX_TILES 24
#endif
#ifndef FLX_SERVER_SHADERS_DEPTH2
#define FLX_SERVER_SHADERS_DEPTH2 2
#endif
#ifndef FLX_SERVER_SHADE_PRIO
#define FLX_SERVER_SHADE_PRIO 0
#endif
#ifndef FLX_SERVER_PRIO
#define FLX_SERVER_PRIO 1
#endif
constexpr uint32_t SV_S = SV_MAX_DEPTH;
enum { RK_SHADE = 0, RK_WALK = 1, RK_READY = 2 };
enum { SC_ALIVE = 0, SC_RING = SC_ALIVE + SV_S , SC_TILEDRY = SC_RING + 9 * SV_S, SC_SAVAIL = SC_TILEDRY + SV_S ,
       SC_SEQ = SC_SAVAIL + SV_S , SC_SLOTP = SC_SEQ + SV_S , SC_ROTLOCK, SC_EXIT, SC_STOPPED,
       SC_STOPAFTER, SC_LASTWORK, SC_NTILES , SC_WORDS = 64 };
static_assert(SC_NTILES + SV_S <= SC_WORDS, "control words");
constexpr uint32_t SC_VIEW_WORDS = 64;

typedef const __attribute__((address_space(4))) ServerKernelArgs *ServerKernelArgsP;
FLX_DEV const ServerArgs &server_args(FrameArgsP p) {
  ServerKernelArgsP q = (ServerKernelArgsP)p;
  asm volatile("" : "+s"(q));
  return *(const ServerArgs *)&q->sa;
}
#define FLX_SERVER_ARGS() FLX_ARGS_OF(ab); const ServerArgs &sa = server_args(ab); (void)sa

template <bool VER, bool THICK>
__global__ __launch_bounds__(FLX_WF_WALK_THREADS, FLX_WF_WAVES_PER_EU) void k_wf_server(ServerKernelArgs , uint32_t ldsCount, uint32_t nTransforms,
                                                                                     uint32_t shadeWaves, uint32_t readyUnits) {
  const FrameArgsP ab = kernel_frame_args();
  constexpr uint32_t WAVES = FLX_WF_WALK_THREADS / 64u;
  const uint32_t WALK_WAVES = WAVES - shadeWaves;
  uint32_t samples, depth, itemsPerSlot, tilesPerSlot;
  { FLX_SERVER_ARGS(); samples = (uint32_t)fr.samples; depth = sa.depth; itemsPerSlot = sa.itemsPerSlot; tilesPerSlot = sa.tilesPerSlot; }
  extern __shared__ float4 ldsAll[];
  float4 *ldsEntries = ldsAll;
  float4 *ldsXf = ldsAll + (size_t)ldsCount * 3u;
  uint32_t *ctl = (uint32_t *)(ldsXf + (size_t)nTransforms * 4u * (VER ? depth : 1u));
  FrameView *lv = (FrameView *)(ctl + SC_WORDS);
  float2 *raysBase = (float2 *)(ctl + SC_WORDS + SC_VIEW_WORDS);
  uint32_t *rings;
  {
    FLX_SERVER_ARGS();
    rings = wb.frameRings + (size_t)blockIdx.x * SV_RINGS * FQ_SIZE;
    for (uint32_t t = threadIdx.x; t < ldsCount * 3u; t += FLX_WF_WALK_THREADS) ldsEntries[t] = sc.walk[t];
    if (!VER)
    for (uint32_t t = threadIdx.x; t < nTransforms * 4u; t += FLX_WF_WALK_THREADS) {
      const uint32_t tr = t >> 2, k = t & 3u, iI = 2u * tr + 1u;
      ldsXf[t] = k < 3u ? sc.rotation[3u * iI + k] : sc.shift[iI];
    }
    if (threadIdx.x < (uint32_t)SC_WORDS) {
      uint32_t v = 0u;
      const uint32_t w = threadIdx.x;
      if (w >= (uint32_t)SC_SEQ && w < (uint32_t)SC_SEQ + SV_S) { const uint32_t slot = w - SC_SEQ; v = sa.seq0 + (slot >= sa.slot0 ? slot - sa.slot0 : slot + depth - sa.slot0); }
      if (w == (uint32_t)SC_SLOTP) v = sa.slot0;
      if (w == (uint32_t)SC_LASTWORK) v = (uint32_t)wall_clock64();
      ctl[w] = v;
    }
  }
  __syncthreads();
  const uint32_t lane = threadIdx.x & 63u;
  const uint32_t wave = threadIdx.x >> 6;
  const uint32_t perTile = samples * 64u;
  WorkCounters cnt = {};

  auto ring = [&](uint32_t kind, uint32_t slot) -> uint32_t * { return rings + (size_t)(kind * SV_S + slot) * FQ_SIZE; };
  auto rctl = [&](uint32_t kind, uint32_t slot) -> uint32_t * { return ctl + SC_RING + 3u * (kind * SV_S + slot); };
  auto slotOf = [&](uint32_t id) -> uint32_t { return (id >= itemsPerSlot ? 1u : 0u) + (id >= 2u * itemsPerSlot ? 1u : 0u); };
  auto slotAt = [&](uint32_t P, uint32_t r) -> uint32_t { const uint32_t s = P + r; return s >= depth ? s - depth : s; };
  auto aliveAll = [&]() -> uint32_t { return fq_load(&ctl[SC_ALIVE]) + fq_load(&ctl[SC_ALIVE + 1]) + fq_load(&ctl[SC_ALIVE + 2]); };
  auto statAdd = [&](int word, unsigned long long v) { FLX_SERVER_ARGS(); if (sa.stats && lane == 0) atomicAdd(sa.stats + word, v); };
  auto worked = [&]() { if (lane == 0) __hip_atomic_store(&ctl[SC_LASTWORK], (uint32_t)wall_clock64(), __ATOMIC_RELAXED, __HIP_MEMORY_SCOPE_WORKGROUP); };
  auto giveUp = [&](uint32_t code) {
    FLX_SERVER_ARGS();
    if (sa.stats && fq_load(&ctl[SC_EXIT]) == 0u) {
      unsigned long long at = SV_DUMP_MAX;
      if (lane == 0) at = atomicAdd(sa.stats + SVS_DUMPS, 1ull);
      at = __shfl(at, 0, 64);
      if (at < (unsigned long long)SV_DUMP_MAX) {
        unsigned long long *d = sa.stats + SV_STAT_WORDS + at * SV_DUMP_WORDS;
// ... 18 lines not shown
      if (lane == 0) { seq = __hip_atomic_load(&sa.mail->posted[slot], __ATOMIC_RELAXED, __HIP_MEMORY_SCOPE_SYSTEM); stop = __hip_atomic_load(&sa.mail->stopAfter, __ATOMIC_RELAXED, __HIP_MEMORY_SCOPE_SYSTEM); }
      if (lane == 0 && stop != 0u) __hip_atomic_store(&sa.relay->stopAfter, stop, __ATOMIC_RELAXED, __HIP_MEMORY_SCOPE_AGENT);
      if (__builtin_amdgcn_readfirstlane(seq) == want) {
        __builtin_amdgcn_fence(__ATOMIC_ACQUIRE, "");
        if (lane < 19u) {
          const uint32_t v = __hip_atomic_load((const uint32_t *)&sa.mail->view[slot] + lane, __ATOMIC_RELAXED, __HIP_MEMORY_SCOPE_SYSTEM);
          __hip_atomic_store((uint32_t *)&sa.relay->view[slot] + lane, v, __ATOMIC_RELAXED, __HIP_MEMORY_SCOPE_AGENT);
        }
        if (VER)
          for (uint32_t t = lane; t < sa.blobWords; t += 64u)
            __hip_atomic_store(&sa.relay->blob[slot][t], __hip_atomic_load(&sa.mail->blob[slot][t], __ATOMIC_RELAXED, __HIP_MEMORY_SCOPE_SYSTEM), __ATOMIC_RELAXED, __HIP_MEMORY_SCOPE_AGENT);
        __builtin_amdgcn_fence(__ATOMIC_RELEASE, "agent");
        asm volatile("s_waitcnt vmcnt(0)" ::: "memory");
        uint32_t again = 0;
        if (lane == 0) again = __hip_atomic_load(&sa.mail->posted[slot], __ATOMIC_ACQUIRE, __HIP_MEMORY_SCOPE_SYSTEM);
        const bool still = __builtin_amdgcn_readfirstlane(again) == want && fq_load(&ctl[SC_SEQ + slot]) == want;
        if (still && lane == 0) __hip_atomic_store(&sa.relay->posted[slot], want, __ATOMIC_RELAXED, __HIP_MEMORY_SCOPE_AGENT);
      }
    }
    uint32_t seq = 0, stop = 0;
    if (lane == 0) { seq = __hip_atomic_load(&sa.relay->posted[slot], __ATOMIC_RELAXED, __HIP_MEMORY_SCOPE_AGENT); stop = __hip_atomic_load(&sa.relay->stopAfter, __ATOMIC_RELAXED, __HIP_MEMORY_SCOPE_AGENT); }
    if (lane == 0 && stop != 0u) __hip_atomic_store(&ctl[SC_STOPAFTER], stop, __ATOMIC_RELAXED, __HIP_MEMORY_SCOPE_WORKGROUP);
    seq = __builtin_amdgcn_readfirstlane(seq);
    if (seq != want) return false;
    __builtin_amdgcn_fence(__ATOMIC_ACQUIRE, "agent");
    if (fq_load(&ctl[SC_SAVAIL + slot]) == 1u) return true;
    if (lane < 19u) ((uint32_t *)&lv[slot])[lane] = __hip_atomic_load((const uint32_t *)&sa.relay->view[slot] + lane, __ATOMIC_RELAXED, __HIP_MEMORY_SCOPE_AGENT);
    if (VER) {
      const uint32_t nRot = nTransforms * 24u, nSh = nTransforms * 8u, ver = blockIdx.x * depth + slot;
      uint32_t *rotW = (uint32_t *)const_cast<float4 *>(sc.rotation) + (size_t)ver * nRot;
      uint32_t *shW = (uint32_t *)const_cast<float4 *>(sc.shift) + (size_t)ver * nSh;
      uint32_t *ltW = (uint32_t *)const_cast<float *>(sc.lights) + (size_t)ver * 6u * sc.n_lights;
      uint32_t *xfW = (uint32_t *)(ldsXf + (size_t)slot * nTransforms * 4u);
      for (uint32_t t = lane; t < sa.blobWords; t += 64u) {
        const uint32_t v = __hip_atomic_load(&sa.relay->blob[slot][t], __ATOMIC_RELAXED, __HIP_MEMORY_SCOPE_AGENT);
        if (t < nRot) {
          rotW[t] = v;
          const uint32_t q = t >> 2, i = q / 3u, k = q - 3u * i;
          if (i & 1u) xfW[((i >> 1) * 4u + k) * 4u + (t & 3u)] = v;
        } else if (t < nRot + nSh) {
          const uint32_t u = t - nRot, i = u >> 2;
          shW[u] = v;
          if (i & 1u) xfW[((i >> 1) * 4u + 3u) * 4u + (u & 3u)] = v;
        } else {
          ltW[t - nRot - nSh] = v;
        }
      }
    }
    __builtin_amdgcn_fence(__ATOMIC_RELEASE, "workgroup");
    if (fq_load(&ctl[SC_SEQ + slot]) != want) return false;
    if (lane == 0) __hip_atomic_store(&ctl[SC_SAVAIL + slot], 1u, __ATOMIC_RELAXED, __HIP_MEMORY_SCOPE_WORKGROUP);
    return true;
  };

  auto makeTile = [&](uint32_t slot, uint32_t r) -> uint32_t {
    if (fq_load(&ctl[SC_TILEDRY + slot]) != 0u) return 2u;
    FLX_SERVER_ARGS();
    uint32_t take = 0, tile = 0;
    if (lane == 0 && fq_load(&ctl[SC_NTILES + slot]) >= sa.tileListCap) {
      if (fq_load(&ctl[SC_SAVAIL + slot]) == 1u && __hip_atomic_load(&sa.slots[slot].tileNext, __ATOMIC_RELAXED, __HIP_MEMORY_SCOPE_AGENT) >= tilesPerSlot)
        __hip_atomic_store(&ctl[SC_TILEDRY + slot], 1u, __ATOMIC_RELAXED, __HIP_MEMORY_SCOPE_WORKGROUP);
    } else
    if (lane == 0 && fq_load(&rctl(RK_READY, slot)[2]) < readyUnits) {
      const uint32_t mySeq = fq_load(&ctl[SC_SEQ + slot]);
      atomicAdd(&ctl[SC_ALIVE + slot], perTile);
      const bool still = fq_load(&ctl[SC_SEQ + slot]) == mySeq && fq_load(&ctl[SC_SAVAIL + slot]) == 1u && fq_load(&ctl[SC_TILEDRY + slot]) == 0u && fq_load(&ctl[SC_SEQ + slot]) == mySeq;
      if (!still || aliveAll() > FQ_ALIVE_MAX - r * (uint32_t)FLX_SERVER_RESERVE) atomicSub(&ctl[SC_ALIVE + slot], perTile);
      else { tile = __hip_atomic_fetch_add(&sa.slots[slot].tileNext, 1u, __ATOMIC_RELAXED, __HIP_MEMORY_SCOPE_AGENT); take = 1; }
    }
    take = __builtin_amdgcn_readfirstlane(take);
    tile = __builtin_amdgcn_readfirstlane(tile);
    if (take == 0u) return 0u;
    if (tile >= tilesPerSlot) {
      if (lane == 0) { __hip_atomic_store(&ctl[SC_TILEDRY + slot], 1u, __ATOMIC_RELAXED, __HIP_MEMORY_SCOPE_WORKGROUP); atomicSub(&ctl[SC_ALIVE + slot], perTile); }
      return 2u;
    }
    tile += slot * tilesPerSlot;
    if (lane == 0) {
      const uint32_t at = atomicAdd(&ctl[SC_NTILES + slot], 1u);
      if (at < sa.tileListCap) sa.tileLists[((size_t)blockIdx.x * SV_S + slot) * sa.tileListCap + at] = tile;
      else __hip_atomic_fetch_or(sa.error, WF_ERR_LIST, __ATOMIC_RELAXED, __HIP_MEMORY_SCOPE_SYSTEM);
    }
    const float4 h = primary_tile<false, true, VER>(ab, tile, lane, cnt, lv);
    const bool runs = shade0_tile<false, true, VER>(ab, tile, lane, h, cnt, lv);
    if (flx_ballot(runs) == 0ull) {
      __builtin_amdgcn_fence(__ATOMIC_RELEASE, "workgroup");
      if (lane == 0) atomicSub(&ctl[SC_ALIVE + slot], perTile);
    } else {
      for (uint32_t s0 = 0; s0 < samples; s0 += 64u)
        fq_push(ring(RK_READY, slot), rctl(RK_READY, slot), s0 + lane < samples, tile * samples + s0 + lane, lane);
    }
    statAdd(SVS_TILES, 1ull);
    return 1u;
  };

  auto tryRotate = [&]() {
    const uint32_t P = fq_load(&ctl[SC_SLOTP]);
    if (!(fq_load(&ctl[SC_SAVAIL + P]) == 1u && fq_load(&ctl[SC_TILEDRY + P]) != 0u && fq_load(&ctl[SC_ALIVE + P]) == 0u)) return;
    uint32_t mine = 0;
    if (lane == 0) mine = atomicCAS(&ctl[SC_ROTLOCK], 0u, 1u) == 0u ? 1u : 0u;
    if (__builtin_amdgcn_readfirstlane(mine) == 0u) return;
    uint32_t ok = 0;
    if (lane == 0) ok = (fq_load(&ctl[SC_SLOTP]) == P && fq_load(&ctl[SC_SAVAIL + P]) == 1u && fq_load(&ctl[SC_TILEDRY + P]) != 0u && fq_load(&ctl[SC_ALIVE + P]) == 0u) ? 1u : 0u;
    if (__builtin_amdgcn_readfirstlane(ok) != 0u) {
      FLX_SERVER_ARGS();
      __builtin_amdgcn_fence(__ATOMIC_ACQUIRE, "workgroup");
      const uint32_t nT = fq_load(&ctl[SC_NTILES + P]) < sa.tileListCap ? fq_load(&ctl[SC_NTILES + P]) : sa.tileListCap;
      const uint32_t *list = sa.tileLists + ((size_t)blockIdx.x * SV_S + P) * sa.tileListCap;
      const size_t stride = (size_t)fr.rows * fr.width;
      for (uint32_t t = 0; t < nT; t++) {
        uint32_t px, k;
        tile8_pixel(fr, list[t], lane, px, k);
        if (px < fr.width && k < fr.rows) {
          const size_t o = (size_t)k * fr.width + px;
          const float4 c = resolve_pixel(fr, wb.hits, wb.sampleRadiance, wb.lastOriginal, o, stride);
          uint32_t row = k - P * fr.frame_rows;
          if (sa.outStripRows) { const uint32_t strip = row / sa.outStripRows; row = strip * sa.outStripStep + (row - strip * sa.outStripRows); }
          if (sa.out8) ((uint32_t *)sa.out[P])[(size_t)row * fr.width + px] = pack_rgba8(c.x, c.y, c.z, c.w);
          else sa.out[P][(size_t)row * fr.width + px] = c;
        }
      }
      if (sa.outSystem) __builtin_amdgcn_fence(__ATOMIC_RELEASE, ""); else
      __builtin_amdgcn_fence(__ATOMIC_RELEASE, "agent");
      asm volatile("s_waitcnt vmcnt(0)" ::: "memory");
      if (lane == 0) {
        const uint32_t seqOld = fq_load(&ctl[SC_SEQ + P]);
        __hip_atomic_store(&ctl[SC_NTILES + P], 0u, __ATOMIC_RELAXED, __HIP_MEMORY_SCOPE_WORKGROUP);
        __hip_atomic_store(&ctl[SC_SEQ + P], seqOld + depth, __ATOMIC_RELAXED, __HIP_MEMORY_SCOPE_WORKGROUP);
        __hip_atomic_store(&ctl[SC_SAVAIL + P], 0u, __ATOMIC_RELAXED, __HIP_MEMORY_SCOPE_WORKGROUP);
        __builtin_amdgcn_fence(__ATOMIC_RELEASE, "workgroup");
        __hip_atomic_store(&ctl[SC_TILEDRY + P], 0u, __ATOMIC_RELAXED, __HIP_MEMORY_SCOPE_WORKGROUP);
        __hip_atomic_store(&ctl[SC_SLOTP], P + 1u >= depth ? 0u : P + 1u, __ATOMIC_RELAXED, __HIP_MEMORY_SCOPE_WORKGROUP);
        const uint32_t before = __hip_atomic_fetch_add(&sa.slots[P].groupsDone, 1u, __ATOMIC_RELAXED, __HIP_MEMORY_SCOPE_AGENT);
        if (before + 1u == gridDim.x) {
          __hip_atomic_store(&sa.slots[P].tileNext, 0u, __ATOMIC_RELAXED, __HIP_MEMORY_SCOPE_AGENT);
          __hip_atomic_store(&sa.slots[P].groupsDone, 0u, __ATOMIC_RELAXED, __HIP_MEMORY_SCOPE_AGENT);
          __builtin_amdgcn_fence(__ATOMIC_RELEASE, "agent");
          asm volatile("s_waitcnt vmcnt(0)" ::: "memory");
          __hip_atomic_store(&sa.mail->done[P], seqOld, __ATOMIC_RELEASE, __HIP_MEMORY_SCOPE_SYSTEM);
          if (sa.stats) atomicAdd(sa.stats + SVS_FRAMES, 1ull);
        }
        if (sa.stats) atomicAdd(sa.stats + SVS_ROTATIONS, 1ull);
      }
    }
    if (lane == 0) __hip_atomic_store(&ctl[SC_ROTLOCK], 0u, __ATOMIC_RELEASE, __HIP_MEMORY_SCOPE_WORKGROUP);
  };

  auto checkExit = [&]() {
    const uint32_t stop = fq_load(&ctl[SC_STOPAFTER]);
    if (stop != 0u && aliveAll() == 0u) {
      uint32_t out = 0;
      if (lane == 0 && atomicCAS(&ctl[SC_ROTLOCK], 0u, 1u) == 0u) {
        const uint32_t P = fq_load(&ctl[SC_SLOTP]);
        out = ((int32_t)(fq_load(&ctl[SC_SEQ + P]) - stop) > 0 && aliveAll() == 0u) ? 1u : 0u;
        if (out) __hip_atomic_store(&ctl[SC_EXIT], 1u, __ATOMIC_RELAXED, __HIP_MEMORY_SCOPE_WORKGROUP);
        __hip_atomic_store(&ctl[SC_ROTLOCK], 0u, __ATOMIC_RELEASE, __HIP_MEMORY_SCOPE_WORKGROUP);
      }
      if (__builtin_amdgcn_readfirstlane(out) != 0u) return;
    }
    FLX_SERVER_ARGS();
    const uint32_t last = fq_load(&ctl[SC_LASTWORK]);
    if ((int32_t)((uint32_t)wall_clock64() - last) > (int32_t)sa.idleExit) giveUp(WF_ERR_SERVER_IDLE);
  };

  auto leave = [&]() {
    __builtin_amdgcn_fence(__ATOMIC_RELEASE, "workgroup");
    uint32_t last = 0;
    if (lane == 0) last = atomicAdd(&ctl[SC_STOPPED], 1u) + 1u == WAVES ? 1u : 0u;
    if (__builtin_amdgcn_readfirstlane(last) == 0u) return;
    FLX_SERVER_ARGS();
    for (uint32_t k = 0; k < 9u; k++)
      if (fq_load(&ctl[SC_RING + 3u * k]) != fq_load(&ctl[SC_RING + 3u * k + 1u]) && lane == 0) __hip_atomic_fetch_or(sa.error, WF_ERR_LEFTOVER, __ATOMIC_RELAXED, __HIP_MEMORY_SCOPE_SYSTEM);
    if (sa.stats && lane == 0) atomicMax(sa.stats + SVS_END, (unsigned long long)wall_clock64());
  };

  if (wave >= WALK_WAVES) {
    uint32_t idle = 0;
    if (FLX_SERVER_SHADE_PRIO) __builtin_amdgcn_s_setprio(FLX_SERVER_SHADE_PRIO);
    const long long tShade0 = wall_clock64();
    long long tTile = 0, tBatch = 0;
    for (;;) {
      if (fq_load(&ctl[SC_EXIT]) != 0u) break;
      tryRotate();
      const uint32_t P = fq_load(&ctl[SC_SLOTP]);
      bool did = false;
      uint32_t nAvail = 0, waiting = 0;
      for (uint32_t r = 0; r < depth; r++) {
        const uint32_t slot = slotAt(P, r);
        if (!sAvail(slot, (idle & 7u) == 0u)) break;
        nAvail = r + 1u;
        waiting += fq_load(&rctl(RK_SHADE, slot)[2]);
      }
      if (nAvail != 0u && waiting != 0u &&
          (waiting >= 64u || idle != 0u || (fq_load(&ctl[SC_TILEDRY + P]) != 0u && fq_load(&rctl(RK_SHADE, P)[2]) != 0u))) {
        uint32_t id = WF_INVALID, got = 0;
        for (uint32_t r = 0; r < nAvail && got < 64u; r++) {
          const uint32_t slot = slotAt(P, r);
          const unsigned long long takers = got == 0u ? ~0ull : (~0ull << got);
          got += fq_pop(ring(RK_SHADE, slot), rctl(RK_SHADE, slot), takers, 64u - got, 1u, lane, id);
        }
        if (got != 0u) {
          const long long tb0 = wall_clock64();
          const bool mine = lane < got && id != WF_INVALID;
          statAdd(SVS_BATCHES, 1ull); statAdd(SVS_BATCH_LANES, got);
          if (mine) shade_path<false, true, VER>(ab, id, cnt, lv);
          const uint32_t slotMine = slotOf(id);
          for (uint32_t sl = 0; sl < depth; sl++) fq_push(ring(RK_WALK, sl), rctl(RK_WALK, sl), mine && slotMine == sl, id, lane);
          tBatch += wall_clock64() - tb0;
          did = true;
        }
      }
      for (uint32_t r = 0; r < nAvail && !did; r++) {
        const long long tt0 = wall_clock64();
        if (makeTile(slotAt(P, r), r) == 1u) { tTile += wall_clock64() - tt0; did = true; }
      }
      if (did) { idle = 0; worked(); continue; }
      checkExit();
      idle++;
      __builtin_amdgcn_s_sleep(8);
    }
    statAdd(SVS_SHADE_TILE_T, (unsigned long long)tTile); statAdd(SVS_SHADE_BATCH_T, (unsigned long long)tBatch); statAdd(SVS_SHADE_TOTAL_T, (unsigned long long)(wall_clock64() - tShade0));
    leave();
    return;
  }

  float2 *myRays = raysBase + (size_t)threadIdx.x * nTransforms * 5u;
  const float4 *walkG; { FLX_ARGS_OF(ab); walkG = pinnedWalkCopy(sc); }
  const float4 *ldsEntriesV = ldsEntries, *walkGV = walkG;
  asm volatile("" : "+v"(ldsEntriesV), "+v"(walkGV));
  WalkLane L;
  walkLaneInit(L);
  uint32_t chunkNext = 0, chunkEnd = 0;
  uint32_t statTrips = 0, statLaneTrips = 0;

  for (;;) {
    const unsigned long long walking = flx_ballot(L.st == P_WALKING);
    const unsigned long long workMask = flx_ballot(L.st == P_DONE || L.st == P_SWITCH);
    const uint32_t parked = 64u - (uint32_t)__popcll(walking);
    bool mayRefill = chunkNext != chunkEnd;
    for (uint32_t s = 0; s < depth && !mayRefill; s++) mayRefill = fq_load(&rctl(RK_WALK, s)[2]) != 0u || fq_load(&rctl(RK_READY, s)[2]) != 0u;
    statTrips += (uint32_t)FLX_WF_INNER; statLaneTrips += (uint32_t)__popcll(walking) * (uint32_t)FLX_WF_INNER;
    if (walking == 0ull || (parked >= (uint32_t)FLX_WF_BATCH && (workMask != 0ull || mayRefill))) {
      uint32_t newId = WF_INVALID;
      bool newFresh = false;
      WalkRecord newRec;
      newRec.q0 = newRec.q1 = newRec.q2 = newRec.q3 = make_float4(0.f, 0.f, 0.f, 0.f);
      const uint32_t P = fq_load(&ctl[SC_SLOTP]);
      {
        const bool want = L.st == P_EMPTY || L.st == P_DONE;
        for (;;) {
          const unsigned long long idle = flx_ballot(want && newId == WF_INVALID);
          if (idle == 0ull) break;
          const bool mineIdle = ((idle >> lane) & 1ull) != 0ull;
          const uint32_t nIdle = (uint32_t)__popcll(idle);
          const uint32_t rk = lane_rank(idle);
          bool got = false, any = false;
          for (uint32_t r = 0; r < depth; r++) {
            const uint32_t slot = slotAt(P, r);
            if (fq_load(&ctl[SC_SAVAIL + slot]) != 1u) break;
            uint32_t id = WF_INVALID;
            if (fq_pop(ring(RK_WALK, slot), rctl(RK_WALK, slot), idle, nIdle, 1u, lane, id) != 0u) {
              if (mineIdle && id != WF_INVALID) newId = id;
              any = flx_ballot(mineIdle && id != WF_INVALID) != 0ull;
              got = true;
              break;
            }
            if (chunkNext == chunkEnd && fq_load(&rctl(RK_SHADE, slot)[2]) < FQ_LIMIT) {
              uint32_t unit = WF_INVALID;
              if (fq_pop(ring(RK_READY, slot), rctl(RK_READY, slot), 1ull, 1u, 1u, lane, unit) != 0u) {
                unit = __builtin_amdgcn_readfirstlane(unit);
                if (unit != WF_INVALID) { chunkNext = unit << 6; chunkEnd = chunkNext + 64u; }
                else if (lane == 0) { FLX_SERVER_ARGS(); atomicSub(&ctl[SC_ALIVE + slot], 64u); __hip_atomic_fetch_or(sa.error, WF_ERR_RING_SLOT, __ATOMIC_RELAXED, __HIP_MEMORY_SCOPE_SYSTEM); }
              }
            }
            if (chunkNext != chunkEnd && slotOf(chunkNext) == slot) {
              const uint32_t avail = chunkEnd - chunkNext;
              const uint32_t take = nIdle < avail ? nIdle : avail;
              if (mineIdle && rk < take) { newId = chunkNext + rk; newFresh = true; }
              chunkNext += take;
              got = true; any = true;
              break;
            }
          }
          if (!got || !any) break;
        }
        if (newId != WF_INVALID) { FLX_ARGS_OF(ab); walkLaneFetchRecord(fr, wb, newId, newFresh, newRec); }
      }
      if (flx_ballot(L.st == P_DONE) != 0ull) {
// ... 97 lines not shown
```

web-ray-tracer_amd/csrc/flx_wavefront.hip:

```cpp
#include <atomic>
#include <mutex>
#include <cstdio>
#include "flx_kernels.h"
#include "flx_kernel_util.h"
#include "flx_wavefront_common.h"
#include "flx_frame_common.h"

namespace flx {


#ifndef FLX_WF_WALK_THREADS
#define FLX_WF_WALK_THREADS 1024
#endif
#ifndef FLX_WF_DRAWS_PER_WAVE
#define FLX_WF_DRAWS_PER_WAVE 16
#endif
#ifndef FLX_WF_PRETRANSFORM
#define FLX_WF_PRETRANSFORM 1
#endif
#ifndef FLX_WF_LDS_TOTAL
#define FLX_WF_LDS_TOTAL (156 * 1024)
#endif
#ifndef FLX_WF_INNER
#define FLX_WF_INNER 8
// ... 568 lines not shown
            }
          }
        }
        chunkNext += take;
      }
      if (COUNT) { const long long tl = clock64(); tLoad += tl - t1; }
      if (st == P_SWITCH) {
        if (flags & RF_NO_CLOSEST) st = P_DONE;
        else { w.mode = 1; st = P_SETUP; }
      }
      if (flx_ballot(st == P_SETUP) != 0ull) {
        if (st == P_SETUP) {
          const bool shadowMode = w.mode == 0;
          const Ray src = shadowMode ? shadowRay : nextRay;
          walkSetupRays(sc, nTransforms, ldsXf, myRays, src, shadowMode);
          w.tR = src; w.cachedTI = 0; w.minLen = shadowMode ? shadowLen : POW32; w.i = (int)sc.walk_root;
          reciprocalOfDir(sc, src.dir, src.origin, w.inv, w.fastDiv);
          st = P_WALKING;
          if (walkFetchP<COUNT>(sc, ldsEntries, ldsCount, myRays, w, cur, cnt)) st = shadowMode ? P_SWITCH : P_DONE;
        }
      }
      if (COUNT) tRefill += clock64() - t1;
      if (flx_ballot(st == P_WALKING) == 0ull) {
        if (itemsLeft || chunkNext != chunkEnd || flx_ballot(st == P_SWITCH || st == P_DONE) != 0ull) continue;
#if FLX_WF_CONSOLIDATE
        if (tailSynced) continue;
#endif
        break;
      }
    }
    long long t2 = COUNT ? clock64() : 0;
#pragma unroll FLX_WF_UNROLL
    for (int it = 0; it < FLX_WF_INNER; it++) {
      if (COUNT) diagIters++;
      if (st == P_WALKING) {
        bool ended = false;
        if (walkIsBoxT(cur)) walkBoxP(w, cur); else ended = walkTriT(w, cur);
        if (!ended) ended = walkFetchP<COUNT>(sc, ldsEntries, ldsCount, myRays, w, cur, cnt);
        if (ended) st = (w.mode == 0) ? P_SWITCH : P_DONE;
      }
#if FLX_DIAG_PAD_SALU
      { uint32_t a = 1, b = 2, c = 3, d = 4;
        for (int k = 0; k < FLX_DIAG_PAD_SALU / 4; k++) asm volatile("s_mov_b32 %0, %1\n s_mov_b32 %1, %2\n s_mov_b32 %2, %3\n s_mov_b32 %3, %0" : "+s"(a), "+s"(b), "+s"(c), "+s"(d) : : "scc"); }
#endif
#if FLX_DIAG_PAD_VALU
      { uint32_t a = lane, b = lane, c = lane, d = lane;
        for (int k = 0; k < FLX_DIAG_PAD_VALU / 4; k++) asm volatile("v_add_u32 %0, %0, 1\n v_add_u32 %1, %1, 1\n v_add_u32 %2, %2, 1\n v_add_u32 %3, %3, 1" : "+v"(a), "+v"(b), "+v"(c), "+v"(d)); }
#endif
    }
    if (COUNT) tInner += clock64() - t2;
  }
#if FLX_WF_CONSOLIDATE
  if (lane == 0) { atomicSub(&tailCtl[TC_LIVE], 1u); if (tailMode) { atomicSub(&tailCtl[TC_TAIL], 1u); atomicAnd(&tailCtl[TC_MASK], ~(1u << (threadIdx.x >> 6))); } }
#endif
  if (outValid) {
    for (uint32_t t = outUsed + lane; t < WF_OUT_CHUNK; t += 64u) listOut[outBase + t] = WF_INVALID;
  }
  if (COUNT && b == 0 && (cnt.closest_visits | cnt.shadow_visits) != 0u) atomicAdd(wb.counters + 23, (unsigned long long)cnt.closest_visits + cnt.shadow_visits);
  flush_counters<COUNT>(cnt, wb.counters);
  if (COUNT && lane == 0) {
    atomicAdd(wb.counters + 8 + 2 * (b < 4 ? b : 3), (unsigned long long)diagIters); atomicAdd(wb.counters + 9 + 2 * (b < 4 ? b : 3), (unsigned long long)diagBatches);
    const unsigned long long life = (unsigned long long)(clock64() - tStart);
    if (b == 0) {
      atomicAdd(wb.counters + 16, (unsigned long long)tFold); atomicAdd(wb.counters + 17, (unsigned long long)tRefill);
      atomicAdd(wb.counters + 18, (unsigned long long)tInner); atomicAdd(wb.counters + 19, life); atomicAdd(wb.counters + 20, 1ull);
      atomicAdd(wb.counters + 21, (unsigned long long)tLoad); atomicAdd(wb.counters + 22, (unsigned long long)tTail);
    }
    if (b < 4) {
      atomicAdd(wb.counters + 24 + 3 * b, life); atomicAdd(wb.counters + 25 + 3 * b, 1ull); atomicMax(wb.counters + 26 + 3 * b, life);
    }
  }
}

#ifndef FLX_FRAME_WALK_PRIO
#define FLX_FRAME_WALK_PRIO 0
#endif
#ifndef FLX_FRAME_SHADE_PRIO
#define FLX_FRAME_SHADE_PRIO 0
#endif
#ifndef FLX_FRAME_SHADERS
#define FLX_FRAME_SHADERS 2
#endif
#ifndef FLX_FRAME_SHADERS_FRONT
#define FLX_FRAME_SHADERS_FRONT 4
#endif
#ifndef FLX_FRAME_PROLOGUE_WAVES
#define FLX_FRAME_PROLOGUE_WAVES 2
#endif
#ifndef FLX_FRAME_GROUPS_PER_CU
#define FLX_FRAME_GROUPS_PER_CU 1
#endif
#ifndef FLX_FRAME_AUTO_MAX_ITEMS
#define FLX_FRAME_AUTO_MAX_ITEMS (64u << 20)
#endif
#ifndef FLX_FRAME_AUTO_MAX_ITEMS_FRONT
#define FLX_FRAME_AUTO_MAX_ITEMS_FRONT (128u << 20)
#endif
template <bool COUNT, bool FRONT, bool STAMP, bool THICK>
__device__ __forceinline__ void wf_frame_body(uint32_t total_items, uint32_t ldsCount, uint32_t nTransforms, uint32_t shadeWaves, uint32_t readyUnits) {
  const uint32_t n = total_items;
  if (n == 0u) return;
  const FrameArgsP argBase = kernel_frame_args();
#define FLX_FRAME_ARGS() FLX_ARGS_OF(argBase)
  const uint32_t WALK_WAVES = FLX_WF_WALK_THREADS / 64u - shadeWaves;
  uint32_t *frameRings; uint32_t samples; bool compactRecs;
  { FLX_FRAME_ARGS(); frameRings = wb.frameRings; samples = (uint32_t)fr.samples; compactRecs = wb.rec0 != nullptr; }
  extern __shared__ float4 ldsAll[];
  float4 *ldsEntries = ldsAll;
  float4 *ldsXf = ldsAll + (size_t)ldsCount * 3u;
  uint32_t *ctl = (uint32_t *)(ldsXf + (size_t)nTransforms * 4u);
  uint32_t *shadeRing = frameRings + (size_t)blockIdx.x * WF_FRAME_RINGS * FQ_SIZE, *walkRing = shadeRing + FQ_SIZE, *readyRing = walkRing + FQ_SIZE;
  constexpr bool front = FRONT;
  const uint32_t perTile = samples * 64u;
  float2 *raysBase = (float2 *)(ctl + FC_WORDS);
  {
    FLX_FRAME_ARGS();
    for (uint32_t t = threadIdx.x; t < ldsCount * 3u; t += FLX_WF_WALK_THREADS) ldsEntries[t] = sc.walk[t];
    for (uint32_t t = threadIdx.x; t < nTransforms * 4u; t += FLX_WF_WALK_THREADS) {
      const uint32_t tr = t >> 2, k = t & 3u, iI = 2u * tr + 1u;
      ldsXf[t] = k < 3u ? sc.rotation[3u * iI + k] : sc.shift[iI];
    }
  }
  if (threadIdx.x < (uint32_t)FC_WORDS) ctl[threadIdx.x] = 0u;
  __syncthreads();
  const uint32_t lane = threadIdx.x & 63u;
  const uint32_t wave = threadIdx.x >> 6;
  WorkCounters cnt = {};

  const uint32_t nTiles = n / perTile;
  auto makeTile = [&]() -> uint32_t {
    if (!FRONT) return 2u;
    FLX_FRAME_ARGS();
    uint32_t take = 0, tile = 0;
    if (lane == 0 && fq_load(&ctl[FC_RQ + 2]) < readyUnits) {
      const uint32_t before = atomicAdd(&ctl[FC_ALIVE], perTile);
      if (before + perTile > FQ_ALIVE_MAX) atomicSub(&ctl[FC_ALIVE], perTile);
      else { tile = atomicAdd(wb.walkQueue, 1u); take = 1; }
    }
    take = __builtin_amdgcn_readfirstlane(take);
    tile = __builtin_amdgcn_readfirstlane(tile);
    if (take == 0u) return 0u;
    if (tile >= nTiles) {
      if (lane == 0) atomicSub(&ctl[FC_ALIVE], perTile);
      return 2u;
    }
    if (wb.tileOrder) tile = __builtin_amdgcn_readfirstlane(wb.tileOrder[tile]);
    tile += wb.item_base / perTile;
    const float4 h = primary_tile<COUNT>(argBase, tile, lane, cnt);
    const bool runs = shade0_tile<COUNT>(argBase, tile, lane, h, cnt);
    if (flx_ballot(runs) == 0ull) {
      if (lane == 0) atomicSub(&ctl[FC_ALIVE], perTile);
    } else {
      for (uint32_t s0 = 0; s0 < samples; s0 += 64u)
        fq_push(readyRing, ctl + FC_RQ, s0 + lane < samples, tile * samples + s0 + lane, lane);
    }
    return 1u;
  };

  if (wave >= WALK_WAVES) {
    uint32_t idle = 0;
    bool frontDone = !front;
    uint32_t inject; { FLX_FRAME_ARGS(); inject = wb.inject; } asm volatile("" : "+s"(inject));
    if (FLX_FRAME_SHADE_PRIO) __builtin_amdgcn_s_setprio(FLX_FRAME_SHADE_PRIO);
    const long long tStartShade = COUNT ? clock64() : 0;
    uint32_t thinMarks = 0;
    for (;;) {
      FLX_FRAME_ARGS();
      const bool dry = fq_load(&ctl[FC_DRY]) != 0u;
      if (COUNT && dry && wave == WALK_WAVES && lane == 0 && thinMarks != 7u) {
        const uint32_t alive = fq_load(&ctl[FC_ALIVE]);
        const unsigned long long now = (unsigned long long)(clock64() - tStartShade);
        for (uint32_t k = 0; k < 3u; k++)
          if ((thinMarks & (1u << k)) == 0u && alive <= (256u >> (2u * k))) { thinMarks |= 1u << k; atomicAdd(wb.counters + 76 + k, now); }
        if (thinMarks == 7u) atomicAdd(wb.counters + 79, 1ull);
      }
      uint32_t id = WF_INVALID;
      const uint32_t got = fq_pop(shadeRing, ctl + FC_SQ, ~0ull, 64u, dry ? 1u : 64u, lane, id);
      if (got == 0u && !frontDone) {
        const uint32_t made = makeTile();
        if (made == 2u) {
          if (lane == 0 && atomicAdd(&ctl[FC_FRONT_DONE], 1u) + 1u == shadeWaves) {
            atomicExch(&ctl[FC_DRY], 1u);
            if (COUNT) {
              const unsigned long long now = (unsigned long long)(clock64() - tStartShade);
              atomicAdd(wb.counters + 60, now); atomicMax(wb.counters + 61, now); atomicAdd(wb.counters + 62, 1ull);
              atomicAdd(wb.counters + 63, (unsigned long long)fq_load(&ctl[FC_ALIVE]));
            }
          }
          frontDone = true;
        }
        if (made != 0u) { idle = 0; continue; }
      }
      if (got == 0u) {
        if (dry && fq_load(&ctl[FC_ALIVE]) == 0u) break;
        if (++idle > (wb.watchdog ? wb.watchdog : FQ_WATCHDOG)) {
          if (lane == 0 && wb.error) __hip_atomic_fetch_or(wb.error, WF_ERR_SHADE_WATCHDOG, __ATOMIC_RELAXED, __HIP_MEMORY_SCOPE_SYSTEM);
          if (COUNT && lane == 0) { for (uint32_t k = 0; k < 8u; k++) atomicMax(wb.counters + 40 + k, (unsigned long long)fq_load(&ctl[k]) + 1ull); atomicAdd(wb.counters + 48, 1ull); }
          break;
        }
        __builtin_amdgcn_s_sleep(8);
        continue;
      }
      idle = 0;
      const bool mine = lane < got && id != WF_INVALID;
      if (flx_ballot(lane < got && id == WF_INVALID) != 0ull && lane == 0 && wb.error) __hip_atomic_fetch_or(wb.error, WF_ERR_RING_SLOT, __ATOMIC_RELAXED, __HIP_MEMORY_SCOPE_SYSTEM);
      if (inject & WF_INJECT_NO_SHADING) continue;
      if (mine) shade_path<COUNT>(argBase, id, cnt);
      fq_push(walkRing, ctl + FC_WQ, mine, id, lane);
    }
    { FLX_FRAME_ARGS(); flush_counters<COUNT>(cnt, wb.counters); }
    return;
  }

  const long long tStart = COUNT ? clock64() : 0;
  if (front && wave < (uint32_t)FLX_FRAME_PROLOGUE_WAVES) while (makeTile() == 1u) {}
  if (FLX_FRAME_WALK_PRIO) __builtin_amdgcn_s_setprio(FLX_FRAME_WALK_PRIO);
  float2 *myRays = raysBase + (size_t)threadIdx.x * nTransforms * 5u;
  const float4 *walkG; { FLX_FRAME_ARGS(); walkG = pinnedWalkCopy(sc); }
#if FLX_WF_FETCH_VBASE
  const float4 *ldsEntriesV = ldsEntries, *walkGV = walkG;
  asm volatile("" : "+v"(ldsEntriesV), "+v"(walkGV));
#define FLX_FETCH_G walkGV
#define FLX_FETCH_L ldsEntriesV
#else
#define FLX_FETCH_G walkG
#define FLX_FETCH_L ldsEntries
#endif
  const uint32_t nWaves = gridDim.x * WALK_WAVES;
  uint32_t lastBase = 0;
  uint32_t inChunk = n / (nWaves * FLX_WF_DRAWS_PER_WAVE);
  inChunk = inChunk < 64u ? 64u : (inChunk > WF_IN_CHUNK ? WF_IN_CHUNK : inChunk);

  long long tBlock = 0, tFoldT = 0, tRefillT = 0, tSetupT = 0, tTrips = 0, tAcqT = 0, tFoldOnlyT = 0; unsigned long long nBlocks = 0, nOuter = 0;
  WalkLane L;
  walkLaneInit(L);
#if FLX_BOX_FALLBACK_COUNT
  L.w.boxTests = L.w.boxExact = 0u;
#endif
  uint32_t chunkNext = 0, chunkEnd = 0;
  bool itemsLeft = true;
  uint32_t idleSpins = 0;

  auto drawChunk = [&]() -> bool {
    FLX_FRAME_ARGS();
    uint32_t *__restrict__ queue = wb.walkQueue;
    if (!itemsLeft) return false;
    if (fq_load(&ctl[FC_SQ + 2]) >= FQ_LIMIT) return false;
    uint32_t want = (n - lastBase) / (nWaves * 2u);
    want = want < 64u ? 64u : (want > inChunk ? inChunk : want);
    uint32_t base0 = 0, room = 1;
    if (lane == 0) {
      const uint32_t before = atomicAdd(&ctl[FC_ALIVE], want);
      if (before + want > FQ_ALIVE_MAX) { atomicSub(&ctl[FC_ALIVE], want); room = 0; }
      else base0 = atomicAdd(queue, want);
    }
    room = __builtin_amdgcn_readfirstlane(room);
    if (room == 0u) return false;
    base0 = __builtin_amdgcn_readfirstlane(base0);
    if (base0 >= n) {
      if (lane == 0) {
        atomicSub(&ctl[FC_ALIVE], want);
        const uint32_t was = atomicExch(&ctl[FC_DRY], 1u);
        if (COUNT && was == 0u) {
          const unsigned long long now = (unsigned long long)(clock64() - tStart);
          atomicAdd(wb.counters + 60, now); atomicMax(wb.counters + 61, now); atomicAdd(wb.counters + 62, 1ull);
          atomicAdd(wb.counters + 63, (unsigned long long)fq_load(&ctl[FC_ALIVE]));
        }
      }
      itemsLeft = false;
      return false;
    }
    const uint32_t have = (base0 + want < n) ? want : n - base0;
    if (have < want && lane == 0) atomicSub(&ctl[FC_ALIVE], want - have);
    lastBase = base0;
    chunkNext = base0; chunkEnd = base0 + have;
      return true;
  };
  auto itemOfQueue = [&](uint32_t q) -> uint32_t {
    FLX_FRAME_ARGS();
    uint32_t id = wb.item_base + q;
    if (wb.tileOrder) { uint32_t tile_, s_; item_tile(fr, id, tile_, s_); id = ((wb.tileOrder[tile_] * (uint32_t)fr.samples + s_) << 6) | (id & 63u); }
    return id;
  };
  for (;;) {
    const unsigned long long walking = flx_ballot(L.st == P_WALKING);
    if (walking != 0ull) idleSpins = 0;
    const unsigned long long workMask = flx_ballot(L.st == P_DONE || L.st == P_SWITCH);
    const uint32_t parked = 64u - (uint32_t)__popcll(walking);
    const bool mayRefill = (front ? fq_load(&ctl[FC_RQ + 2]) != 0u : itemsLeft) || chunkNext != chunkEnd || fq_load(&ctl[FC_WQ + 2]) != 0u;
    if (COUNT) nOuter++;
// ... 299 lines not shown
```

Before: 13060.

## Add cosine sample table, single-light reservoir shortcut, angle tables and shader count change

```diff
diff --git a/include/flx_reservoir_first.h b/include/flx_reservoir_first.h
--- /dev/null
+++ b/include/flx_reservoir_first.h
@@ -0,0 +1,30 @@
+#ifndef FLX_RESERVOIR_FIRST_H
+#define FLX_RESERVOIR_FIRST_H
+
+#include "flx_math.h"
+
+#define FLX_NOISE_PHI 1.61803398874989484820459f
+
+FLX_HD float flx_noise_y_arg(float random_seed, float nx, float ny, float seed) {
+  float d = nx * 12.9898f + ny * 78.233f;
+  float k = seed + random_seed * FLX_NOISE_PHI;
+  return d + 59.0f * k;
+}
+FLX_HD float flx_noise_y_from_arg(float a) { return flx_fract(flx_sin(a) * 43758.5453f) * 2.0f - 1.0f; }
+
+FLX_HD int flx_first_light_taken_literal(float a, float w) {
+  float y = flx_noise_y_from_arg(a);
+  return flx_abs(y) * w <= w;
+}
+FLX_HD int flx_first_light_taken(float a, float w) {
+  if (!(flx_abs(a) <= 1048576.0f)) return 0;
+  if (w == flx_inff()) {
+#if defined(__HIP_DEVICE_COMPILE__)
+    asm volatile("" : "+v"(a));
+#endif
+    return flx_first_light_taken_literal(a, w);
+  }
+  return w < flx_inff();
+}
+
+#endif
diff --git a/web-ray-tracer_amd/csrc/flx_api.hip b/web-ray-tracer_amd/csrc/flx_api.hip
--- a/web-ray-tracer_amd/csrc/flx_api.hip
+++ b/web-ray-tracer_amd/csrc/flx_api.hip
@@ -302,6 +302,18 @@
   return FLX_OK;
 }
 flx_status flx_angle_table(flx_context *ctx, DeviceScene &sc) { return angle_table(ctx, sc); }
+
+static flx_status cos_table(flx_context *ctx, WavefrontBuffers &wb) {
+  if (!ctx->cos_sample_made || !ctx->d_cos_sample) {
+    flx_status es = ctx->d_cos_sample.ensure(ctx, WF_COS_SAMPLES);
+    if (es) return es;
+    launch_cos_sample(ctx->d_cos_sample, WF_COS_SAMPLES, ctx->stream);
+    FLX_HIP(ctx, hipGetLastError());
+    ctx->cos_sample_made = true;
+  }
+  wb.cosSample = ctx->d_cos_sample; wb.cosSampleCount = WF_COS_SAMPLES;
+  return FLX_OK;
+}
 
 flx_status flx_run_frame(flx_context *ctx, const DeviceScene &sc, const DeviceFrame &fr, float4 *d_out, const GBufferPtrs &gb) {
   { flx_status ss = flx_server_stop(ctx); if (ss) return ss; }
@@ -382,6 +394,10 @@
       FLX_HIP(ctx, hipMemsetAsync(ctx->d_tile_time, 0, (size_t)tiles * sizeof(float), ctx->stream));
     }
     const size_t listSlice = std::min(ctx->d_live[0].capacity(), ctx->d_live[1].capacity()) / (size_t)groups;
+    WavefrontBuffers wbTables;
+    { flx_status es = cos_table(ctx, wbTables); if (es) return es; }
+    DeviceScene scW = sc;
+    if (FLX_FRAME_ANGLE_TABLE && front && (!(adaptive && front) || FLX_THIN_ANGLE_TABLE)) { flx_status es = angle_table(ctx, scW); if (es) return es; }
     if (groups > 1) {
       FLX_HIP(ctx, hipEventRecord(ctx->ev_fork, ctx->stream));
       for (int g = 1; g < groups; g++) FLX_HIP(ctx, hipStreamWaitEvent(ctx->aux_stream[g - 1], ctx->ev_fork, 0));
@@ -403,10 +419,11 @@
       wb.counts = ctx->d_wfcounts + (size_t)g * 2 * (WF_MAX_BOUNCES + 2); wb.walkQueue = wb.counts + (WF_MAX_BOUNCES + 2);
       wb.item_base = t0 * perTile; wb.item_count = (t1 - t0) * perTile;
       wb.hits = ctx->d_hits; wb.sampleRadiance = ctx->d_samples; wb.lastOriginal = ctx->d_last; wb.counters = cnt;
+      wb.cosSample = wbTables.cosSample; wb.cosSampleCount = wbTables.cosSampleCount;
       hipStream_t st = g == 0 ? ctx->stream : ctx->aux_stream[g - 1];
       const uint32_t cusWalk = (ctx->comm && (ctx->twin || ctx->is_twin) && cus > 4u * FLX_COMM_RESERVED_CUS) ? cus - FLX_COMM_RESERVED_CUS : cus;
       WalkLdsLaunch lds;
-      const int ran = launch_wavefront(sc, fr, wb, cusWalk, cnt != nullptr, organisationNow, g == 0 ? ctx->ev_k0 : nullptr, g == 0 ? ctx->ev_k1 : nullptr, st, &lds);
+      const int ran = launch_wavefront(scW, fr, wb, cusWalk, cnt != nullptr, organisationNow, g == 0 ? ctx->ev_k0 : nullptr, g == 0 ? ctx->ev_k1 : nullptr, st, &lds);
       FLX_HIP(ctx, hipGetLastError());
       if (ran == -2) return fail(ctx, FLX_ERR_DEVICE, "the walk kernels need 156 KB of dynamic LDS and hipFuncSetAttribute refused it on this device");
       if (ran < 0) return fail(ctx, FLX_ERR_DEVICE, "internal: the frame kernel was to trace the primary rays but does not take this frame");
@@ -1097,6 +1114,11 @@
     if ((s = server_allocate(ctx, frOne, depth))) return s;
     const size_t P1 = (size_t)frOne.rows * frOne.width;
     ctx->sv_out_pixels = P1;
+    WavefrontBuffers wb = {};
+    if ((s = cos_table(ctx, wb))) return s;
+    DeviceScene scL = sc;
+    const bool ver = ctx->sv_want_ver && server_versions_fit(ctx);
+    if (FLX_SERVER_ANGLE_TABLE && !ver && (s = angle_table(ctx, scL))) return s;
     FLX_HIP(ctx, hipStreamSynchronize(ctx->stream));
     ctx->sv_counter += 16u;
     if (ctx->sv_counter < 16u) ctx->sv_counter = 16u;
@@ -1105,7 +1127,6 @@
     FLX_HIP(ctx, hipMemsetAsync(ctx->d_sv_slots, 0, SV_MAX_DEPTH * sizeof(ServerSlot), ctx->sv_stream));
     FLX_HIP(ctx, hipMemsetAsync(ctx->d_sv_relay, 0, sizeof(ServerMail), ctx->sv_stream));
     FLX_HIP(ctx, hipMemsetAsync(ctx->d_sv_stats, 0, SV_STAT_TOTAL * sizeof(unsigned long long), ctx->sv_stream));
-    WavefrontBuffers wb = {};
     wb.rec = ctx->d_rec; wb.rec0 = ctx->d_rec0; wb.pix0 = ctx->d_pix0;
     wb.frameRings = ctx->d_sv_rings; wb.front = 1u;
     wb.error = ctx->d_dev_error; wb.watchdog = 0u; wb.inject = 0u;
@@ -1130,8 +1151,6 @@
     sa.stats = ctx->d_sv_stats;
     uint32_t cusWalk = cus > 4u * FLX_SERVER_RESERVED_CUS ? cus - FLX_SERVER_RESERVED_CUS : cus;
     if (ctx->sv_groups && ctx->sv_groups < cusWalk) cusWalk = ctx->sv_groups;
-    const bool ver = ctx->sv_want_ver && server_versions_fit(ctx);
-    DeviceScene scL = sc;
     if (ver) {
       const size_t versions = (size_t)cusWalk * depth;
       sa.blobWords = server_blob_words(ctx->n_transforms, ctx->n_lights);
diff --git a/web-ray-tracer_amd/csrc/flx_context.h b/web-ray-tracer_amd/csrc/flx_context.h
--- a/web-ray-tracer_amd/csrc/flx_context.h
+++ b/web-ray-tracer_amd/csrc/flx_context.h
@@ -126,6 +126,8 @@
   uint32_t geometry_version = 0;
   uint32_t transforms_version = 0;
   int angle_table = 1;
+  DeviceBuffer<float> d_cos_sample;
+  bool cos_sample_made = false;
   DeviceBuffer<float4> d_out;
   DeviceBuffer<float4> d_gb[6];
   DeviceBuffer<uint32_t> d_planes[13];
diff --git a/web-ray-tracer_amd/csrc/flx_device.h b/web-ray-tracer_amd/csrc/flx_device.h
--- a/web-ray-tracer_amd/csrc/flx_device.h
+++ b/web-ray-tracer_amd/csrc/flx_device.h
@@ -5,6 +5,7 @@
 #include <stdint.h>
 
 #include "flx_math.h"
+#include "flx_reservoir_first.h"
 
 #define FLX_DEV __device__ __forceinline__
 
@@ -343,6 +344,10 @@
   bool markId;
 };
 
+#ifndef FLX_SHADE_FIRST_LIGHT
+#define FLX_SHADE_FIRST_LIGHT 1
+#endif
+template <bool FIRST = false>
 FLX_DEV void reservoirPick(const DeviceScene &sc, const DeviceFrame &fr, PixelState &ps, const Material &material, const Ray &ray,
                            f4 randomVec, f3 N, f3 smoothNormal, float geometryOffset, bool dontFilter, int i, ShadeOut &so) {
   f3 localColor = F3(0.0f, 0.0f, 0.0f);
@@ -351,9 +356,13 @@
   int reservoirNum = 0;
   float reservoirWeight = 0.0f;
   f3 reservoirLightDir = F3(0.0f, 0.0f, 0.0f);
-  f4 n0 = noise(ps.seed, randomVec.z, randomVec.w, BIAS);
-  float lastRandomX = n0.x, lastRandomY = n0.y;
   const int size = (int)sc.n_lights;
+  const bool oneLight = FIRST && size <= 1;
+  float lastRandomX = 0.0f, lastRandomY = 0.0f;
+  if (!oneLight) {
+    f4 n0 = noise(ps.seed, randomVec.z, randomVec.w, BIAS);
+    lastRandomX = n0.x; lastRandomY = n0.y;
+  }
   for (int j = 0; j < size; j++) {
     const float *lt = sc.lights + 6 * j + ps.lightBase;
     float strength = lt[3], variation = lt[4];
@@ -365,7 +374,9 @@
     localColor = localColor + colorForLight;
     float weight = length(colorForLight);
     totalWeight += weight;
-    if (flx_abs(lastRandomY) * totalWeight <= weight) {
+    const bool taken = oneLight ? flx_first_light_taken(flx_noise_y_arg(ps.seed, randomVec.z, randomVec.w, BIAS), weight) != 0
+                                : flx_abs(lastRandomY) * totalWeight <= weight;
+    if (taken) {
       reservoirNum = j;
       reservoirWeight = weight;
       reservoirLightDir = dir;
@@ -417,7 +428,7 @@
                           mul(rTI, F3(a0.x, a0.y, a0.z)), mul(rTI, F3(a0.w, a1.x, a1.y)), mul(rTI, F3(a1.z, a1.w, a2.x)));
 }
 
-template <bool COUNT>
+template <bool COUNT, bool TABLE = (FLX_ANGLE_TABLE != 0)>
 FLX_DEV void shadeSurface(const DeviceScene &sc, const DeviceFrame &fr, const Hit &hit, const Ray &ray, f3 lastHitPoint, SurfaceCtx &sf,
                           WorkCounters &cnt) {
   if (COUNT) cnt.shades++;
@@ -440,7 +451,7 @@
                                  (n0.y * uvw.x + n1.y * uvw.y) + n2.y * uvw.z,
                                  (n0.z * uvw.x + n1.z * uvw.y) + n2.z * uvw.z));
   f3 angleTan;
-  if (FLX_ANGLE_TABLE && sc.angle_tan) { const float4 t = sc.angle_tan[hit.triangleId]; angleTan = F3(t.x, t.y, t.z); }
+  if (TABLE && sc.angle_tan) { const float4 t = sc.angle_tan[hit.triangleId]; angleTan = F3(t.x, t.y, t.z); }
   else angleTan = triangleAngleTan(t0v, t1v, t2v, n0, n1, n2);
   sf.geometryOffset = dot(diffs * angleTan, uvw);
   float bu = (a2.y * uvw.x + a2.w * uvw.y) + a3.y * uvw.z;
@@ -457,6 +468,7 @@
   sf.F0 = sf.material.albedo * sf.BRDF;
 }
 
+template <bool FIRST = false>
 FLX_DEV void shadeSample(const DeviceScene &sc, const DeviceFrame &fr, const SurfaceCtx &sf, PixelState &ps, PathState &p, f3 camera, float cosSampleN,
                          int i, ShadeOut &so) {
   const float fi = (float)i;
@@ -496,7 +508,7 @@
   }
 
   if (i == 1) ps.firstRayLength = flx_min(length(p.ray.origin - p.lastHitPoint) / length(p.lastHitPoint - camera), ps.firstRayLength);
-  reservoirPick(sc, fr, ps, material, p.ray, randomVec, roughNormal * (-sf.signDir), smoothNormal * (-sf.signDir), sf.geometryOffset, p.dontFilter, i, so);
+  reservoirPick<FIRST>(sc, fr, ps, material, p.ray, randomVec, roughNormal * (-sf.signDir), smoothNormal * (-sf.signDir), sf.geometryOffset, p.dontFilter, i, so);
   if (isSolid) {
     p.ray.dir = normalize(mix(reflect(p.ray.dir, smoothNormal), randomSpheareVec, sf.roughnessBRDF));
   } else {
@@ -505,12 +517,12 @@
   }
 }
 
-template <bool COUNT>
+template <bool COUNT, bool TABLE = (FLX_ANGLE_TABLE != 0), bool FIRST = false>
 FLX_DEV void bounceShade(const DeviceScene &sc, const DeviceFrame &fr, PixelState &ps, PathState &p, f3 camera, float cosSampleN, int i,
                          ShadeOut &so, WorkCounters &cnt) {
   SurfaceCtx sf;
-  shadeSurface<COUNT>(sc, fr, p.hit, p.ray, p.lastHitPoint, sf, cnt);
-  shadeSample(sc, fr, sf, ps, p, camera, cosSampleN, i, so);
+  shadeSurface<COUNT, TABLE>(sc, fr, p.hit, p.ray, p.lastHitPoint, sf, cnt);
+  shadeSample<FIRST>(sc, fr, sf, ps, p, camera, cosSampleN, i, so);
 }
 
 #ifndef FLX_BOX_FALLBACK_COUNT
diff --git a/web-ray-tracer_amd/csrc/flx_frame_common.h b/web-ray-tracer_amd/csrc/flx_frame_common.h
--- a/web-ray-tracer_amd/csrc/flx_frame_common.h
+++ b/web-ray-tracer_amd/csrc/flx_frame_common.h
@@ -27,7 +27,7 @@
 #define FLX_WF_DRAWS_PER_WAVE 16
 #endif
 #ifndef FLX_FRAME_SHADERS_FRONT
-#define FLX_FRAME_SHADERS_FRONT 4
+#define FLX_FRAME_SHADERS_FRONT 3
 #endif
 #ifndef FLX_WF_MAX_TRANSFORMS
 #define FLX_WF_MAX_TRANSFORMS 4
@@ -44,10 +44,25 @@
 FLX_DEV FrameArgsP kernel_frame_args() { return (FrameArgsP)__builtin_amdgcn_kernarg_segment_ptr(); }
 #define FLX_ARGS_OF(ab) const FrameArgs &A_ = frame_args(ab); const DeviceScene &sc = A_.sc; const DeviceFrame &fr = A_.fr; const WavefrontBuffers &wb = A_.wb; (void)sc; (void)fr; (void)wb
 
+#ifndef FLX_SHADE_COS_TABLE
+#define FLX_SHADE_COS_TABLE 1
+#endif
+typedef const __attribute__((address_space(4))) float *ConstFloatP;
+template <bool SHORT>
+FLX_DEV float sample_cos_uniform(const WavefrontBuffers &wb, uint32_t s) {
+  if (SHORT && FLX_SHADE_COS_TABLE && s < wb.cosSampleCount) return ((ConstFloatP)(uintptr_t)wb.cosSample)[s];
+  return flx_cos((float)s);
+}
+template <bool SHORT>
+FLX_DEV float sample_cos(const WavefrontBuffers &wb, uint32_t s) {
+  if (SHORT && FLX_SHADE_COS_TABLE && s < wb.cosSampleCount) return wb.cosSample[s];
+  return flx_cos((float)s);
+}
+
 template <bool VER>
 FLX_DEV uint32_t scene_version_of(const DeviceFrame &fr, uint32_t frameIdx) { return VER ? blockIdx.x * fr.frames + frameIdx : 0u; }
 
-template <bool COUNT, bool LV = false, bool VER = false>
+template <bool COUNT, bool LV = false, bool VER = false, bool TABLE = (FLX_ANGLE_TABLE != 0), bool SHORT = false>
 FLX_DEV bool shade0_tile(FrameArgsP ab, uint32_t tile, uint32_t lane, float4 h, WorkCounters &cnt, const FrameView *lv = nullptr) {
   uint32_t S, frameIdx, lightBase = 0;
   int tri;
@@ -77,7 +92,7 @@
     pr.origin = camera;
     pr.dir = primary_dir_v(fr, view_at<LV>(fr, lv, frameIdx), px, py_gl, ndcX, ndcY, viewDepthPerS);
     const WorkCounters before = cnt;
-    shadeSurface<COUNT>(sc, fr, hit, pr, camera, sf, cnt);
+    shadeSurface<COUNT, TABLE>(sc, fr, hit, pr, camera, sf, cnt);
     if (COUNT) {
       cnt.shades = before.shades + (cnt.shades - before.shades) * S;
       cnt.atlas_texels = before.atlas_texels + (cnt.atlas_texels - before.atlas_texels) * S;
@@ -107,9 +122,9 @@
     p.lastHitPoint = camera;
     p.dontFilter = true;
     p.importancyFactor = F3(1.0f, 1.0f, 1.0f);
-    const float cosSampleN = flx_cos((float)s);
+    const float cosSampleN = sample_cos_uniform<SHORT>(wb, s);
     ShadeOut so;
-    shadeSample(sc, fr, sf, ps, p, camera, cosSampleN, 0, so);
+    shadeSample<SHORT && FLX_SHADE_FIRST_LIGHT>(sc, fr, sf, ps, p, camera, cosSampleN, 0, so);
     const int flags = (p.dontFilter ? RF_DONT_FILTER : 0) | (so.needShadow ? RF_NEED_SHADOW : 0) | (so.shadowedNoWalk ? RF_SHADOWED_NO_WALK : 0) |
                       (nextBounceRuns(fr, 0, p.importancyFactor, ps.originalColor) ? 0 : RF_NO_CLOSEST);
     if (compact) {
@@ -169,7 +184,7 @@
   return h;
 }
 
-template <bool COUNT, bool LV = false, bool VER = false>
+template <bool COUNT, bool LV = false, bool VER = false, bool TABLE = (FLX_ANGLE_TABLE != 0), bool SHORT = false>
 FLX_DEV void shade_path(FrameArgsP ab, uint32_t pathId, WorkCounters &cnt, const FrameView *lv = nullptr) {
   FLX_ARGS_OF(ab);
   float4 *rec = wb.rec + (size_t)pathId * 8;
@@ -198,9 +213,9 @@
   float viewDepthPerS;
   (void)primary_dir_v(fr, view_at<LV>(fr, lv, frameIdx), px, py_gl, ps.ndc_x, ps.ndc_y, viewDepthPerS);
   ps.seed = view_at<LV>(fr, lv, frameIdx).random_seed;
-  const float cosSampleN = flx_cos((float)s);
+  const float cosSampleN = sample_cos<SHORT>(wb, s);
   ShadeOut so;
-  bounceShade<COUNT>(sc, fr, ps, p, camera, cosSampleN, pb, so, cnt);
+  bounceShade<COUNT, TABLE, SHORT && FLX_SHADE_FIRST_LIGHT>(sc, fr, ps, p, camera, cosSampleN, pb, so, cnt);
   const int flags = (p.dontFilter ? RF_DONT_FILTER : 0) | (so.needShadow ? RF_NEED_SHADOW : 0) | (so.shadowedNoWalk ? RF_SHADOWED_NO_WALK : 0) |
                     (nextBounceRuns(fr, pb, p.importancyFactor, ps.originalColor) ? 0 : RF_NO_CLOSEST);
   rec[0] = make_float4(p.ray.origin.x, p.ray.origin.y, p.ray.origin.z, __int_as_float(flags));
diff --git a/web-ray-tracer_amd/csrc/flx_kernels.h b/web-ray-tracer_amd/csrc/flx_kernels.h
--- a/web-ray-tracer_amd/csrc/flx_kernels.h
+++ b/web-ray-tracer_amd/csrc/flx_kernels.h
@@ -5,6 +5,15 @@
 
 #ifndef FLX_PATHS_ANGLE_TABLE
 #define FLX_PATHS_ANGLE_TABLE 1
+#endif
+#ifndef FLX_FRAME_ANGLE_TABLE
+#define FLX_FRAME_ANGLE_TABLE 1
+#endif
+#ifndef FLX_SERVER_ANGLE_TABLE
+#define FLX_SERVER_ANGLE_TABLE 1
+#endif
+#ifndef FLX_THIN_ANGLE_TABLE
+#define FLX_THIN_ANGLE_TABLE 0
 #endif
 #define FLX_FAST_BOX_BOUND 5.764607523034235e17f
 namespace flx {
@@ -46,6 +55,8 @@
   uint32_t tileCostPrimary;
   const uint32_t *tileOrder;
   unsigned long long *tileCost;
+  const float *cosSample = nullptr;
+  uint32_t cosSampleCount = 0;
 };
 struct FrameArgs { DeviceScene sc; DeviceFrame fr; WavefrontBuffers wb; };
 constexpr uint32_t WF_FRAME_RING = 16384;
@@ -65,6 +76,8 @@
 void launch_taa(const uint32_t *const planes[9], uint32_t *out8, int W, int H, hipStream_t stream);
 void launch_quantize(const float4 *src, uint32_t *dst, size_t n, hipStream_t stream);
 void launch_angle_tan(const DeviceScene &sc, float4 *out, hipStream_t stream);
+constexpr uint32_t WF_COS_SAMPLES = 64;
+void launch_cos_sample(float *out, uint32_t n, hipStream_t stream);
 void launch_filter_chain(const FilterPlanes &pl, float4 *out, int W, int H, int hdr, hipStream_t stream);
 struct TemporalPass {
   const float4 *color, *color_ip, *location_id, *original_id, *original_color, *id;
diff --git a/web-ray-tracer_amd/csrc/flx_kernels.hip b/web-ray-tracer_amd/csrc/flx_kernels.hip
--- a/web-ray-tracer_amd/csrc/flx_kernels.hip
+++ b/web-ray-tracer_amd/csrc/flx_kernels.hip
@@ -581,6 +581,14 @@
   hipLaunchKernelGGL(k_angle_tan, dim3((sc.n_entries + 255u) / 256u), dim3(256), 0, stream, s, out);
 }
 
+__global__ __launch_bounds__(64) void k_cos_sample(float *__restrict__ out, uint32_t n) {
+  const uint32_t s = blockIdx.x * 64u + threadIdx.x;
+  if (s < n) out[s] = flx_cos((float)s);
+}
+void launch_cos_sample(float *out, uint32_t n, hipStream_t stream) {
+  if (n) hipLaunchKernelGGL(k_cos_sample, dim3((n + 63u) / 64u), dim3(64), 0, stream, out, n);
+}
+
 uint64_t path_item_count64(const DeviceFrame &fr) {
   return (uint64_t)((fr.width + 7u) >> 3) * ((fr.rows + 7u) >> 3) * (uint64_t)fr.samples * 64u;
 }
diff --git a/web-ray-tracer_amd/csrc/flx_server.hip b/web-ray-tracer_amd/csrc/flx_server.hip
--- a/web-ray-tracer_amd/csrc/flx_server.hip
+++ b/web-ray-tracer_amd/csrc/flx_server.hip
@@ -10,7 +10,7 @@
 #define FLX_SERVER_RELAY_GROUPS 16
 #endif
 #ifndef FLX_SERVER_SHADERS
-#define FLX_SERVER_SHADERS FLX_FRAME_SHADERS_FRONT
+#define FLX_SERVER_SHADERS 4
 #endif
 #ifndef FLX_SERVER_SHADERS_DEPTH2_MAX_TILES
 #define FLX_SERVER_SHADERS_DEPTH2_MAX_TILES 24
@@ -195,7 +195,7 @@
       else __hip_atomic_fetch_or(sa.error, WF_ERR_LIST, __ATOMIC_RELAXED, __HIP_MEMORY_SCOPE_SYSTEM);
     }
     const float4 h = primary_tile<false, true, VER>(ab, tile, lane, cnt, lv);
-    const bool runs = shade0_tile<false, true, VER>(ab, tile, lane, h, cnt, lv);
+    const bool runs = shade0_tile<false, true, VER, FLX_SERVER_ANGLE_TABLE && !VER, true>(ab, tile, lane, h, cnt, lv);
     if (flx_ballot(runs) == 0ull) {
       __builtin_amdgcn_fence(__ATOMIC_RELEASE, "workgroup");
       if (lane == 0) atomicSub(&ctl[SC_ALIVE + slot], perTile);
@@ -316,7 +316,7 @@
           const long long tb0 = wall_clock64();
           const bool mine = lane < got && id != WF_INVALID;
           statAdd(SVS_BATCHES, 1ull); statAdd(SVS_BATCH_LANES, got);
-          if (mine) shade_path<false, true, VER>(ab, id, cnt, lv);
+          if (mine) shade_path<false, true, VER, FLX_SERVER_ANGLE_TABLE && !VER, true>(ab, id, cnt, lv);
           const uint32_t slotMine = slotOf(id);
           for (uint32_t sl = 0; sl < depth; sl++) fq_push(ring(RK_WALK, sl), rctl(RK_WALK, sl), mine && slotMine == sl, id, lane);
           tBatch += wall_clock64() - tb0;
diff --git a/web-ray-tracer_amd/csrc/flx_wavefront.hip b/web-ray-tracer_amd/csrc/flx_wavefront.hip
--- a/web-ray-tracer_amd/csrc/flx_wavefront.hip
+++ b/web-ray-tracer_amd/csrc/flx_wavefront.hip
@@ -674,7 +674,7 @@
 #define FLX_FRAME_SHADERS 2
 #endif
 #ifndef FLX_FRAME_SHADERS_FRONT
-#define FLX_FRAME_SHADERS_FRONT 4
+#define FLX_FRAME_SHADERS_FRONT 3
 #endif
 #ifndef FLX_FRAME_PROLOGUE_WAVES
 #define FLX_FRAME_PROLOGUE_WAVES 2
@@ -703,6 +703,7 @@
   uint32_t *ctl = (uint32_t *)(ldsXf + (size_t)nTransforms * 4u);
   uint32_t *shadeRing = frameRings + (size_t)blockIdx.x * WF_FRAME_RINGS * FQ_SIZE, *walkRing = shadeRing + FQ_SIZE, *readyRing = walkRing + FQ_SIZE;
   constexpr bool front = FRONT;
+  constexpr bool ANGLE_TABLE = FLX_FRAME_ANGLE_TABLE && FRONT && (!STAMP || FLX_THIN_ANGLE_TABLE);
   const uint32_t perTile = samples * 64u;
   float2 *raysBase = (float2 *)(ctl + FC_WORDS);
   {
@@ -739,7 +740,7 @@
     if (wb.tileOrder) tile = __builtin_amdgcn_readfirstlane(wb.tileOrder[tile]);
     tile += wb.item_base / perTile;
     const float4 h = primary_tile<COUNT>(argBase, tile, lane, cnt);
-    const bool runs = shade0_tile<COUNT>(argBase, tile, lane, h, cnt);
+    const bool runs = shade0_tile<COUNT, false, false, ANGLE_TABLE, true>(argBase, tile, lane, h, cnt);
     if (flx_ballot(runs) == 0ull) {
       if (lane == 0) atomicSub(&ctl[FC_ALIVE], perTile);
     } else {
@@ -797,7 +798,7 @@
       const bool mine = lane < got && id != WF_INVALID;
       if (flx_ballot(lane < got && id == WF_INVALID) != 0ull && lane == 0 && wb.error) __hip_atomic_fetch_or(wb.error, WF_ERR_RING_SLOT, __ATOMIC_RELAXED, __HIP_MEMORY_SCOPE_SYSTEM);
       if (inject & WF_INJECT_NO_SHADING) continue;
-      if (mine) shade_path<COUNT>(argBase, id, cnt);
+      if (mine) shade_path<COUNT, false, false, ANGLE_TABLE, true>(argBase, id, cnt);
       fq_push(walkRing, ctl + FC_WQ, mine, id, lane);
     }
     { FLX_FRAME_ARGS(); flush_counters<COUNT>(cnt, wb.counters); }
```

Result: faster. 13530, median of 6 (+3.6%).
